# PaulTFLi/Machine-Learning-Replications

Hardware: AMD Instinct MI355X
Metric: train_rows_per_sec (higher is better)
Workload: dtype fp32

## Files before the change

### machine-learning-replications_amd/models/imputer.py

```python
from __future__ import annotations

import os

import numpy as np
import torch

from .base import Estimator, as_tensor

SLOTS = 8
MFMA_FILTER = os.environ.get("HFENS_KNN_MFMA", "auto")
MFMA_MIN_PAIRS = 1 << 24
EXACT = __import__("os").environ.get("HFENS_KNN_EXACT", "1") != "0"
KNN_DEBUG = __import__("os").environ.get("HFENS_KNN_DEBUG", "0") == "1"
DEVICE_PLAN = __import__("os").environ.get("HFENS_KNN_DEVICE_PLAN", "1") != "0"
LAST_REFINE: list = []
REFINE_CAP_MIN = 1 << 18
REFINE_CAP_PER_ROW = 16


def _refine_debug(work, cap, nr, Mx):
    o = 4 * cap + 8 * nr * SLOTS + 2 * nr
    LAST_REFINE.append((nr, int(work[o]), int(work[o + 8]), int(work[o + 9]), int(work[o + 4]), float(Mx[0])))


def _masks_u64(miss: torch.Tensor) -> torch.Tensor:
    F = miss.shape[1]
    w = (2 ** torch.arange(F, dtype=torch.int64, device=miss.device))
    bits = (miss.to(torch.int64) * w).sum(1)
    return bits


class KNNImputer(Estimator):
    _param_names = ("missing_values", "n_neighbors", "weights", "metric", "copy")

    def __init__(self, missing_values=np.nan, n_neighbors=5, weights="uniform", metric="nan_euclidean",
                 copy=True):
        self.missing_values = missing_values
        self.n_neighbors = n_neighbors
        self.weights = weights
        self.metric = metric
        self.copy = copy

    def fit(self, X):
        X = as_tensor(X)
        self._fit_X = X
        self._mask_fit = torch.isnan(X)
        self._valid = ~self._mask_fit.all(0)
        fx = torch.where(self._mask_fit, torch.zeros_like(X), X)
        cnt = (~self._mask_fit).sum(0).clamp(min=1)
        self._col_mean = fx.sum(0) / cnt
        self._keep_host = None
        return self

    def _keep(self):
        if self._keep_host is None:
            self._keep_host = np.nonzero(self._valid.cpu().numpy())[0].astype(np.int64)
        return self._keep_host

    def fit_transform(self, X):
        return self.fit(X).transform(X)

    def transform(self, X):
        return self.transform_many([X])[0]

    def transform_many(self, Xs, streams=None, defer=False):
        Xs = [as_tensor(X, device=self._fit_X.device).clone() for X in Xs]
        if Xs and Xs[0].is_cuda and self.n_neighbors == 1:
            if DEVICE_PLAN and EXACT and Xs[0].shape[1] <= 64:
                return self._impute_planned_many(Xs, streams, defer)
            return self._impute_device_many(Xs, streams, defer)
        if defer:
            done = self.transform_many(Xs)
            return done, (lambda: done)
        for X in Xs:
            miss = torch.isnan(X)
            rows = torch.nonzero(miss.any(1)).squeeze(1)
            if rows.numel() > 0:
                self._impute_host(X, miss, rows)
        return [X[:, self._valid] for X in Xs]

    def _fit_prep(self):
        pr = getattr(self, "_prep", None)
        if pr is None or pr[0] is not self._fit_X:
            D = torch.where(self._mask_fit, torch.zeros_like(self._fit_X), self._fit_X)
            center = self._col_mean
            D32 = (D - center).where(~self._mask_fit, torch.zeros_like(D)).to(torch.float32).contiguous()
            dm = _masks_u64(self._mask_fit).contiguous()
            D64 = D.to(torch.float64).contiguous()
            dmax = D32.abs().amax(0) if D32.numel() else torch.zeros(D32.shape[1], device=D.device)
            pr = self._prep = (self._fit_X, D32, dm, D64, dmax)
        return pr[1], pr[2]

    def _fit_prep64(self):
        self._fit_prep()
        return self._prep[3], self._prep[4]

    def _impute_planned_many(self, Xs, streams, defer=False):
        from .smo import _to_dev
        from ..utils.timing import hmark
        dev = Xs[0].device
        F = Xs[0].shape[1]
        keep_h = self._keep()
        keep = None if keep_h.shape[0] == F else _to_dev(keep_h, dev)
        D32, dm = self._fit_prep()
        D64, dmax = self._fit_prep64()
        main = torch.cuda.current_stream(dev)
        ready = torch.cuda.Event()
        ready.record(main)
        out, jobs = [], []
        for i, X in enumerate(Xs):
            st = streams[i] if streams is not None and streams[i] is not None else None
            if st is None:
                self._impute_planned(X, D32, dm, D64, dmax)
                out.append(X if keep is None else X.index_select(1, keep))
                hmark("imp_main_enqueued")
            else:
                def job(i=i, X=X, st=st):
                    st.wait_event(ready)
                    for t in (X, D32, dm, D64, dmax, self._fit_X, self._col_mean) + ((keep,) if keep is not None else ()):
                        t.record_stream(st)
                    with torch.cuda.device(dev), torch.cuda.stream(st):
                        self._impute_planned(X, D32, dm, D64, dmax)
                        out[i] = X if keep is None else X.index_select(1, keep)
                out.append(None)
                jobs.append(job)
        if not defer:
            for job in jobs:
                job()
            return out
        state = {"done": False}

        def run():
            if not state["done"]:
                for job in jobs:
                    job()
                state["done"] = True
            return out
        return out, run

    def _impute_planned(self, X, D32, dm, D64, dmax):
        from .. import ops
        E = ops.ext()
        n, F = X.shape
        if n == 0:
            return
        dev = X.device
        s = ops.stream_ptr(dev)
        G = -(-F // SLOTS)
        Xc = X if X.is_contiguous() else X.contiguous()
        i64, i32 = torch.int64, torch.int32
        rows = torch.empty(n, dtype=i64, device=dev)
        rbits = torch.empty(n, dtype=i64, device=dev)
        slot = torch.empty(G, n, SLOTS, dtype=i32, device=dev)
        R32 = torch.empty(n, F, dtype=torch.float32, device=dev)
        R64 = torch.empty(n, F, dtype=torch.float64, device=dev)
        small = torch.empty(F + 1 + 4 + (n + 255) // 256, dtype=i32, device=dev)
        colmax, Mx, cnt, bcnt = small[:F], small[F:F + 1], small[F + 1:F + 5], small[F + 5:]
        E.knn_plan_dev(Xc.data_ptr(), n, F, self._col_mean.data_ptr(), dmax.data_ptr(), rows.data_ptr(),
                       rbits.data_ptr(), slot.data_ptr(), G, R32.data_ptr(), R64.data_ptr(), colmax.data_ptr(),
                       Mx.data_ptr(), cnt.data_ptr(), bcnt.data_ptr(), s)
        best = torch.empty(G, n, SLOTS, dtype=i64, device=dev)
        alt = torch.empty(n, SLOTS, dtype=i32, device=dev)
        cap = max(REFINE_CAP_MIN, REFINE_CAP_PER_ROW * n, 1)
        work = torch.empty(4 * cap + n * SLOTS * 8 + 2 * n + 12, dtype=i32, device=dev)
        nd = D32.shape[0]
        mf = None
        use_mf = MFMA_FILTER == "1" or (MFMA_FILTER == "auto" and n * nd >= MFMA_MIN_PAIRS)
        if use_mf and F <= 48 and nd > 0:
            wd = np.zeros(1, dtype=np.int64)
            E.knn_mfma_item_words(F, wd.ctypes.data)
            mf = (torch.empty(nd * int(wd[0]), dtype=torch.int32, device=dev), torch.empty(nd, dtype=torch.float32, device=dev))
            E.knn_mfma_prep(D32.data_ptr(), dm.data_ptr(), nd, F, mf[0].data_ptr(), mf[1].data_ptr(), s)
        for g in range(G):
            if mf is not None:
                E.knn_donors_mfma(R32.data_ptr(), rbits.data_ptr(), n, D32.data_ptr(), dm.data_ptr(), nd, F,
                                  slot[g].data_ptr(), best[g].data_ptr(), alt.data_ptr(), cnt.data_ptr(), g * SLOTS,
                                  mf[0].data_ptr(), mf[1].data_ptr(), s)
            else:
                E.knn_donors(R32.data_ptr(), rbits.data_ptr(), n, D32.data_ptr(), dm.data_ptr(), nd, F,
                             slot[g].data_ptr(), best[g].data_ptr(), alt.data_ptr(), cnt.data_ptr(), g * SLOTS, s)
            E.knn_refine(R32.data_ptr(), rbits.data_ptr(), n, D32.data_ptr(), dm.data_ptr(), nd, F,
                         slot[g].data_ptr(), best[g].data_ptr(), alt.data_ptr(), R64.data_ptr(), D64.data_ptr(),
                         Mx.data_ptr(), work.data_ptr(), cap, cnt.data_ptr(), g * SLOTS,
                         mf[0].data_ptr() if mf is not None else 0, mf[1].data_ptr() if mf is not None else 0, s)
            if KNN_DEBUG:
                _refine_debug(work, cap, n, Mx)
        fx = self._fit_X if self._fit_X.is_contiguous() else self._fit_X.contiguous()
        E.knn_apply(Xc.data_ptr(), n, F, rows.data_ptr(), slot.data_ptr(), best.data_ptr(), fx.data_ptr(),
                    self._col_mean.data_ptr(), cnt.data_ptr(), s)
        if Xc is not X:
            X.copy_(Xc)

    def _impute_device_many(self, Xs, streams, defer=False):
        F = Xs[0].shape[1]
        if F > 64:
            raise ValueError("KNNImputer device path supports at most 64 features")
        from ..utils.timing import hmark
        host = torch.cat([_masks_u64(torch.isnan(X)) for X in Xs] + [self._valid.to(torch.int64)]).cpu().numpy()
        hmark("imp_masks_read")
        bits_all = host[:-F].view(np.uint64)
        from .smo import _to_dev
        dev = Xs[0].device
        keep = _to_dev(np.nonzero(host[-F:])[0].astype(np.int64), dev)
        D32, dm = self._fit_prep()
        main = torch.cuda.current_stream(dev)
        ready = torch.cuda.Event()
        ready.record(main)
        off, out, jobs = 0, [], []
        for i, X in enumerate(Xs):
            bits = bits_all[off:off + X.shape[0]]
            off += X.shape[0]
            st = streams[i] if streams is not None and streams[i] is not None else None
            if st is None:
                self._impute_device(X, bits, D32, dm)
                out.append(X.index_select(1, keep))
                hmark("imp_main_enqueued")
            else:
                def job(i=i, X=X, bits=bits, st=st):
                    st.wait_event(ready)
                    for t in (X, keep, D32, dm, self._fit_X, self._col_mean):
                        t.record_stream(st)
                    with torch.cuda.device(dev), torch.cuda.stream(st):
                        self._impute_device(X, bits, D32, dm)
                        out[i] = X.index_select(1, keep)
                out.append(None)
                jobs.append(job)
        if not defer:
            for job in jobs:
                job()
            return out
        state = {"done": False}

        def run():
            if not state["done"]:
                for job in jobs:
                    job()
                state["done"] = True
            return out
        return out, run

    def _impute_device(self, X, bits, D32, dm):
        from .. import ops
        E = ops.ext()
        n, F = X.shape
        dev = X.device
        dims = np.zeros(4, dtype=np.int64)
        bits = np.ascontiguousarray(bits, dtype=np.uint64)
        E.knn_plan_host(bits.ctypes.data, n, F, SLOTS, 0, 0, dims.ctypes.data)
        nr, nc, nslot = (int(v) for v in dims[:3])
        if nr == 0:
            return
        cap = 2 * nr + nr * nslot + 3 * nc
        hb = torch.empty(cap, dtype=torch.int64, pin_memory=True)
        E.knn_plan_host(bits.ctypes.data, n, F, SLOTS, hb.data_ptr(), cap, dims.ctypes.data)
        if int(dims[3]) != 0 or int(dims[0]) != nr:
            raise RuntimeError(f"knn_plan_host: work-list buffer of {cap} words rejected (dims {dims.tolist()})")
        center = self._col_mean
        from ..utils.timing import hmark
        hmark("imp_plan")
        sizes = [nr, nr, nr * nslot, nc, nc, nc]
        buf = hb[:sum(sizes)].to(dev, non_blocking=True)
        o = np.concatenate([[0], np.cumsum(sizes)])
        rows, rm, slot_dev, flat, r_idx, c_idx = (buf[o[i]:o[i + 1]] for i in range(6))
        hmark("imp_h2d")
        Rm = ((rm[:, None] >> torch.arange(F, device=dev)) & 1) != 0
        slot_dev = slot_dev.view(nr, nslot).to(torch.int32)
        Xr = X.index_select(0, rows)
        R32 = torch.where(Rm, torch.zeros_like(Xr), Xr - center).to(torch.float32).contiguous()
        rm = rm.contiguous()
        best = torch.empty(nr, nslot, dtype=torch.int64, device=dev)
        alt = torch.empty(nr, SLOTS, dtype=torch.int32, device=dev)
        if EXACT:
            D64, dmax = self._fit_prep64()
            R64 = torch.where(Rm, torch.zeros_like(Xr), Xr).to(torch.float64).contiguous()
            Mx = torch.linalg.vector_norm(torch.maximum(dmax, R32.abs().amax(0)).to(torch.float64)).reshape(1)
            Mx = Mx.to(torch.float32).contiguous()
            cap = max(REFINE_CAP_MIN, REFINE_CAP_PER_ROW * nr, 1)
            work = torch.empty(4 * cap + nr * SLOTS * 8 + 2 * nr + 12, dtype=torch.int32, device=dev)
        for s0 in range(0, nslot, SLOTS):
            slot = slot_dev[:, s0:s0 + SLOTS].contiguous()
            blk = best[:, s0:s0 + SLOTS] if nslot == SLOTS else torch.empty(slot.shape, dtype=torch.int64, device=dev)
            E.knn_donors(R32.data_ptr(), rm.data_ptr(), nr, D32.data_ptr(), dm.data_ptr(),
                         D32.shape[0], F, slot.data_ptr(), blk.data_ptr(), alt.data_ptr(), 0, 0, ops.stream_ptr(dev))
            if EXACT:
                E.knn_refine(R32.data_ptr(), rm.data_ptr(), nr, D32.data_ptr(), dm.data_ptr(), D32.shape[0], F,
                             slot.data_ptr(), blk.data_ptr(), alt.data_ptr(), R64.data_ptr(), D64.data_ptr(),
                             Mx.data_ptr(), work.data_ptr(), cap, 0, 0, 0, 0, ops.stream_ptr(dev))
                if KNN_DEBUG:
                    _refine_debug(work, cap, nr, Mx)
            if nslot != SLOTS:
                best[:, s0:s0 + SLOTS] = blk
        hmark("imp_knn_launched")
        b = best.view(-1).index_select(0, flat)
        donor = torch.where(b == -1, torch.full_like(b, -1), b & 0xFFFFFFFF)
        vals = torch.where(donor >= 0, self._fit_X[donor.clamp(min=0), c_idx], self._col_mean[c_idx])
        X.index_put_((r_idx, c_idx), vals)

    def _impute_host(self, X, miss, rows):
        fit = self._fit_X
        mf = self._mask_fit
        F = X.shape[1]
        D = torch.where(mf, torch.zeros_like(fit), fit)
        pres_f = (~mf).to(torch.float64)
        step = max(1, (1 << 24) // max(1, fit.shape[0] * F))
        for s in range(0, rows.numel(), step):
            rr = rows[s:s + step]
            R = X[rr]
            mr = torch.isnan(R)
            Rz = torch.where(mr, torch.zeros_like(R), R)
            pres_r = (~mr).to(torch.float64)
            both = pres_r[:, None, :] * pres_f[None, :, :]
            diff = Rz[:, None, :] - D[None, :, :]
            sq = both * (diff * diff)
            d2 = sq[..., 0].clone()
            for f in range(1, F):
                d2 = d2 + sq[..., f]
            common = both.sum(-1)
            dist = torch.where(common > 0, d2 * F / common.clamp(min=1),
                               torch.full_like(d2, float("inf")))
            for j, r in enumerate(rr.tolist()):
                for c in torch.nonzero(mr[j]).squeeze(1).tolist():
                    cand = ~mf[:, c]
                    dd = torch.where(cand, dist[j], torch.full_like(dist[j], float("inf")))
                    k = min(self.n_neighbors, int(cand.sum()))
                    if k == 0 or not torch.isfinite(dd).any():
                        X[r, c] = self._col_mean[c]
                        continue
                    if k == 1:
                        X[r, c] = fit[int(torch.argmin(dd)), c]
                        continue
                    vals, idx = torch.topk(-dd, k)
                    ok = torch.isfinite(vals)
                    X[r, c] = fit[idx[ok], c].mean()
```

### machine-learning-replications_amd/ops/csrc/decls.inc

```
#if defined(HFENS_DECLS)
#define HFENS_OP(name, sig) void name sig;
#elif defined(HFENS_DEFS)
#define HFENS_OP(name, sig) m.def(#name, &hfens::name);
#endif
HFENS_OP(gbdt_apply_prep, (int B, int n, int F, int NN, uintptr_t bins, uintptr_t y, uintptr_t w,
                           uintptr_t raw, uintptr_t g, uintptr_t h, uintptr_t node, uintptr_t prev_feat,
                           uintptr_t prev_blo, uintptr_t prev_value, uintptr_t prev_r2,
                           uintptr_t dev_acc, uintptr_t cur_r2, double lr, double qscale,
                           double dscale, uintptr_t wt, double subsample, uintptr_t seeds,
                           long long row_off, int stage, uintptr_t stream))
HFENS_OP(gbdt_hist, (int B, int n, int F, uintptr_t bins, uintptr_t nbins, int max_nb, uintptr_t g,
                     uintptr_t h, uintptr_t w, uintptr_t node, int node0, int NL, uintptr_t hist,
                     double qscale, uintptr_t stream))
HFENS_OP(gbdt_split, (int B, int F, int NN, uintptr_t hist, uintptr_t nbins, uintptr_t lo_val,
                      uintptr_t hi_val, int node0, int NL, int last_level, double min_leaf_q,
                      double min_split_q, double qscale, uintptr_t feat, uintptr_t blo, uintptr_t thr,
                      uintptr_t value, uintptr_t stats, uintptr_t r2, uintptr_t stream))
HFENS_OP(gbdt_route, (int B, int n, int NN, uintptr_t bins, uintptr_t g, uintptr_t w, uintptr_t node,
                      uintptr_t feat, uintptr_t blo, uintptr_t r2, int node0, int NL, double qscale,
                      uintptr_t stream))
HFENS_OP(gbdt_stumps_fused, (int B, int n, int F, int T, uintptr_t bins, uintptr_t nbins, int hist_len,
                             uintptr_t lo_val, uintptr_t hi_val, uintptr_t y, uintptr_t w, uintptr_t raw,
                             uintptr_t g, uintptr_t h, uintptr_t wt, uintptr_t seeds, long long row_off,
                             double subsample, uintptr_t feat, uintptr_t blo, uintptr_t thr, uintptr_t value,
                             uintptr_t stats, uintptr_t r2, uintptr_t dev, uintptr_t bagw, double lr,
                             double qscale, double dscale, double min_leaf_q, double min_split_q,
                             uintptr_t stream))
HFENS_OP(l1_qp_cd, (int B, int F1, uintptr_t H, uintptr_t g, uintptr_t w, uintptr_t penal, double lam,
                    int max_sweeps, double tol, uintptr_t d_out, uintptr_t stream))
HFENS_OP(logreg_fused, (int B, int n, int F1, uintptr_t X, uintptr_t s, uintptr_t ypm, uintptr_t penal, double C,
                        int l1, int max_outer, uintptr_t Z, uintptr_t Xd, uintptr_t W, uintptr_t iters,
                        uintptr_t stream))
HFENS_OP(logreg_coop, (int B, int members, int n, int F1, uintptr_t X, uintptr_t s, uintptr_t ypm, uintptr_t penal,
                       double C, int l1, int max_outer, uintptr_t Z, uintptr_t Xd, uintptr_t W, uintptr_t iters,
                       uintptr_t xchg, uintptr_t err, uintptr_t stream))
HFENS_OP(lasso_cd_path, (int P, int F, int A, uintptr_t G, uintptr_t q, uintptr_t yy, uintptr_t nrows,
                         uintptr_t alphas, int max_iter, double tol, uintptr_t coefs, uintptr_t gaps,
                         uintptr_t iters, uintptr_t stream))
HFENS_OP(gram_rbf_batch, (uintptr_t Z, int F, uintptr_t probs, int P, int max_l, uintptr_t K,
                          uintptr_t stream))
HFENS_OP(smo_batch, (uintptr_t probs, int P, int max_l, uintptr_t K, uintptr_t alpha, double eps,
                     long long max_iter, uintptr_t rho, uintptr_t iters, uintptr_t gap, uintptr_t prof,
                     uintptr_t stream))
HFENS_OP(coop_resident_blocks, (uintptr_t out))
HFENS_OP(smo_coop_batch, (uintptr_t probs, int P, int W, int max_S, uintptr_t K, uintptr_t maps,
                          uintptr_t alpha, uintptr_t xchg, double eps, long long max_iter, uintptr_t rho,
                          uintptr_t iters, uintptr_t gap, uintptr_t err, uintptr_t prof, uintptr_t stream))
HFENS_OP(smo_coop_otf_batch, (uintptr_t probs, int P, int W, int F, int max_S, uintptr_t zcat, uintptr_t alpha,
                              uintptr_t xchg, double eps, long long max_iter, uintptr_t rho, uintptr_t iters,
                              uintptr_t gap, uintptr_t err, uintptr_t stream))
HFENS_OP(platt_batch,(uintptr_t probs, int P, uintptr_t part, int S, uintptr_t rowk, uintptr_t rho,
                       uintptr_t consts, uintptr_t srcmap, uintptr_t dec, uintptr_t AB, uintptr_t coop_bar,
                       uintptr_t coop_part, uintptr_t stream))
HFENS_OP(knn_mfma_item_words, (int F, uintptr_t out))
HFENS_OP(knn_mfma_prep, (uintptr_t D, uintptr_t dmask, int nd, int F, uintptr_t items, uintptr_t ny, uintptr_t stream))
HFENS_OP(knn_donors_mfma, (uintptr_t R, uintptr_t rmask, int nr, uintptr_t D, uintptr_t dmask, int nd, int F,
                           uintptr_t slot_col, uintptr_t best, uintptr_t alt, uintptr_t cnt, int s0, uintptr_t items,
                           uintptr_t ny, uintptr_t stream))
HFENS_OP(knn_donors, (uintptr_t R, uintptr_t rmask, int nr, uintptr_t D, uintptr_t dmask, int nd, int F,
                      uintptr_t slot_col, uintptr_t best, uintptr_t alt, uintptr_t cnt, int s0, uintptr_t stream))
HFENS_OP(knn_plan_host, (uintptr_t bits_, long long n, int F, int slots, uintptr_t out_, long long cap,
                         uintptr_t dims_))
HFENS_OP(knn_refine, (uintptr_t R, uintptr_t rmask, int nr, uintptr_t D, uintptr_t dmask, int nd, int F,
                      uintptr_t slot_col, uintptr_t best, uintptr_t alt, uintptr_t R64, uintptr_t D64, uintptr_t Mx,
                      uintptr_t work, long long cap, uintptr_t cnt, int s0, uintptr_t items, uintptr_t ny,
                      uintptr_t stream))
HFENS_OP(weighted_moments, (uintptr_t X, int n, int F, uintptr_t W, uintptr_t V, int P, uintptr_t Gpart,
                            uintptr_t apart, uintptr_t vpart, uintptr_t stream))
HFENS_OP(svc_oof, (uintptr_t dec, uintptr_t model, uintptr_t rho, uintptr_t AB, uintptr_t rows, uintptr_t meta,
                   int ld, int col, int n, uintptr_t stream))
HFENS_OP(svm_dec_batch, (uintptr_t zcat, uintptr_t coef, uintptr_t hcat, int F, uintptr_t probs, int P,
                         int max_h, int S, uintptr_t part, uintptr_t counts, uintptr_t stream))
HFENS_OP(svm_sv_compact, (uintptr_t zcat, uintptr_t coef, int F, uintptr_t probs, int P, uintptr_t zc, uintptr_t cc,
                          uintptr_t counts, uintptr_t stream))
HFENS_OP(libsvm_perm, (int l, long long seed, uintptr_t out_ptr))
HFENS_OP(svc_expand_host, (uintptr_t y_ptr, long long n, long long seed, uintptr_t out_ptr, uintptr_t meta_ptr))
HFENS_OP(sklearn_stump_ranks, (int T, int F, uintptr_t seeds_ptr, uintptr_t constant_ptr, uintptr_t ranks_ptr))
HFENS_OP(wsyrk_f64, (uintptr_t Phi, uintptr_t d, long long n, int r, uintptr_t part, long long part_len, uintptr_t S,
                     uintptr_t stream))
HFENS_OP(wsyrk_f32, (uintptr_t Phi, uintptr_t d, long long n, int r, uintptr_t part, long long part_len, uintptr_t S,
                     uintptr_t stream))
HFENS_OP(wsyrk_f64x, (uintptr_t Phi, uintptr_t d, long long n, int r, uintptr_t part, long long part_len, uintptr_t S,
                      uintptr_t stream))
HFENS_OP(phi_gemv, (uintptr_t Phi, uintptr_t W, long long n, int r, int k, uintptr_t Y, uintptr_t stream))
HFENS_OP(fill_dev, (uintptr_t out, long long n, uintptr_t src, uintptr_t stream))
HFENS_OP(ipm_max_step, (uintptr_t v0, uintptr_t d0, uintptr_t v1, uintptr_t d1, uintptr_t v2, uintptr_t d2,
                        uintptr_t v3, uintptr_t d3, double s0, double s1, double s2, double s3, long long n,
                        uintptr_t out, uintptr_t stream))
HFENS_OP(scale_rows_f32, (uintptr_t P, uintptr_t d, long long n, int r, uintptr_t out, uintptr_t stream))
HFENS_OP(ipm_resid, (uintptr_t c, uintptr_t a, uintptr_t y, uintptr_t P, int sp, uintptr_t b, uintptr_t nu, uintptr_t mu,
                     long long n, uintptr_t s, uintptr_t rd, uintptr_t stream))
HFENS_OP(ipm_pred, (uintptr_t a, uintptr_t s, uintptr_t nu, uintptr_t mu, uintptr_t rd, uintptr_t y, long long n,
                    uintptr_t Dinv, uintptr_t Dinv2, uintptr_t rnu, uintptr_t rmu, uintptr_t H2, uintptr_t stream))
HFENS_OP(ipm_corr, (uintptr_t a, uintptr_t s, uintptr_t nu, uintptr_t mu, uintptr_t da, uintptr_t dnu, uintptr_t dmu,
                    uintptr_t rd, uintptr_t tau, long long n, uintptr_t rnu, uintptr_t rmu, uintptr_t h, uintptr_t stream))
HFENS_OP(ipm_minv_pre, (uintptr_t Dinv, uintptr_t y, uintptr_t U, int k, long long n, uintptr_t du, uintptr_t V,
                        uintptr_t stream))
HFENS_OP(ipm_minv_post, (uintptr_t Dinv, uintptr_t y, uintptr_t du, uintptr_t P, int k, long long n, uintptr_t out,
                         uintptr_t stream))
HFENS_OP(ipm_update, (uintptr_t a, uintptr_t nu, uintptr_t mu, uintptr_t da, uintptr_t dnu, uintptr_t dmu, uintptr_t t,
                      long long n, uintptr_t a2, uintptr_t nu2, uintptr_t mu2, uintptr_t stream))
HFENS_OP(ipm_dirs, (uintptr_t Mh, int smh, uintptr_t My, int smy, uintptr_t db, uintptr_t rnu, uintptr_t rmu,
                    uintptr_t nu, uintptr_t mu, uintptr_t a, uintptr_t s, long long n, uintptr_t da, uintptr_t dnu,
                    uintptr_t dmu, uintptr_t stream))
HFENS_OP(ipm_gondzio_rhs, (uintptr_t a, uintptr_t s, uintptr_t nu, uintptr_t mu, uintptr_t da, uintptr_t dnu,
                           uintptr_t dmu, uintptr_t alpha, uintptr_t tau, long long n, uintptr_t ta, uintptr_t ts,
                           uintptr_t rhs, uintptr_t stream))
HFENS_OP(ipm_gondzio_apply, (uintptr_t Mh, int smh, uintptr_t My, int smy, uintptr_t dbc, uintptr_t da,
                             uintptr_t dnu, uintptr_t dmu, uintptr_t ta, uintptr_t ts, uintptr_t nu, uintptr_t mu,
                             uintptr_t a, uintptr_t s, long long n, uintptr_t nda, uintptr_t ndnu, uintptr_t ndmu,
                             uintptr_t stream))
HFENS_OP(ipm_select3, (uintptr_t ok, uintptr_t x0, uintptr_t x1, uintptr_t x2, long long n, uintptr_t y0,
                       uintptr_t y1, uintptr_t y2, uintptr_t stream))
HFENS_OP(phi_gemv_f32, (uintptr_t Phi, uintptr_t W, long long n, int r, int k, uintptr_t Y, uintptr_t stream))
HFENS_OP(phit_f32, (uintptr_t Phi, uintptr_t V, long long n, int r, int k, uintptr_t part, long long part_len,
                    uintptr_t out, uintptr_t stream))
HFENS_OP(scaler_batch, (uintptr_t X, long long n, int F, uintptr_t rows, uintptr_t offs, int K, long long max_rows,
                        uintptr_t part, uintptr_t mean, uintptr_t var, uintptr_t Z, uintptr_t stream))
HFENS_OP(chol_spd, (uintptr_t S, int r, uintptr_t L, uintptr_t sc, uintptr_t info, uintptr_t stream))
HFENS_OP(chol_spd_mw, (uintptr_t S, int r, uintptr_t L, uintptr_t sc, uintptr_t info, uintptr_t work, uintptr_t PT,
                       uintptr_t stream))
HFENS_OP(chol_solve, (uintptr_t L, uintptr_t sc, int r, int k, uintptr_t B, uintptr_t stream))
HFENS_OP(gbdt_stage_tick, (uintptr_t t_dev, uintptr_t stream))
HFENS_OP(gbdt_stump_stage, (int t, int B, int n, int F, int T, uintptr_t bins, long long ldb, uintptr_t nbins, int hist_len,
                            uintptr_t lo_val, uintptr_t hi_val, uintptr_t y, uintptr_t w, uintptr_t raw,
                            uintptr_t wt, uintptr_t seeds, long long row_off, double subsample, uintptr_t comm,
                            uintptr_t feat, uintptr_t blo, uintptr_t thr, uintptr_t value, uintptr_t stats,
                            uintptr_t r2, uintptr_t dev, uintptr_t bagw, uintptr_t frank, uintptr_t partials,
                            long long partials_len, double lr, double qscale, double dscale,
                            double min_leaf_q, double min_split_q, uintptr_t prof, uintptr_t t_dev,
                            int tick_in_reduce, int persist, uintptr_t bar, uintptr_t err, uintptr_t stream))
HFENS_OP(stack_infer, (uintptr_t X, int x_f64, long long n, int F, int mp, int T, int K, double ngl2e,
                       double svc_b, double probA, double probB, double gb_init, double gb_lr,
                       double lr_b, double mw0, double mw1, double mw2, double mb, uintptr_t mean,
                       uintptr_t inv_scale, uintptr_t svt, uintptr_t sn, uintptr_t coef,
                       uintptr_t nodes, uintptr_t values, uintptr_t lr_w, uintptr_t st_off,
                       uintptr_t st_pairs, double st_base, uintptr_t out, int grid, uintptr_t stream))
HFENS_OP(stack_coalition, (uintptr_t X, long long n, uintptr_t BG, long long B, int F, int mp, int T, int K,
                           double ngl2e, double svc_b, double probA, double probB, double gb_init,
                           double gb_lr, double lr_b, double mw0, double mw1, double mw2, double mb,
                           uintptr_t mean, uintptr_t inv_scale, uintptr_t svt, uintptr_t sn, uintptr_t coef,
                           uintptr_t nodes, uintptr_t values, uintptr_t lr_w, uintptr_t st_off,
                           uintptr_t st_pairs, double st_base, uintptr_t v, int grid, uintptr_t stream))
HFENS_OP(shapley_reduce, (uintptr_t v, long long n, int F, uintptr_t w, uintptr_t phi, uintptr_t stream))
HFENS_OP(ws_init, (uintptr_t probs, int P, int max_l, uintptr_t zcat, int F, uintptr_t zn, uintptr_t alpha,
                   uintptr_t G, uintptr_t states, uintptr_t keys, long long n, uintptr_t hist, uintptr_t gkey,
                   uintptr_t stream))
HFENS_OP(cascade_where, (uintptr_t tab, int Q, long long max_len, uintptr_t where, uintptr_t stream))
HFENS_OP(ws_seed, (uintptr_t probs, int P, int max_l, uintptr_t zcat, int F, uintptr_t zn, uintptr_t aseed,
                   uintptr_t alpha, uintptr_t G, uintptr_t keys, long long n, uintptr_t gkey, uintptr_t stream))
HFENS_OP(ws_steps, (uintptr_t probs, int P, int max_l, uintptr_t zcat, int F, uintptr_t zn, uintptr_t alpha,
                    uintptr_t G, uintptr_t states, uintptr_t wsz, uintptr_t wsn, uintptr_t wdc, uintptr_t wsprev,
                    uintptr_t wsidx, uintptr_t keys, long long n, uintptr_t gkey, double eps, int max_outer, int max_inner,
                    double inner_frac, int n_iter, uintptr_t prof, int inner_threads, int q, uintptr_t stream))
HFENS_OP(ws_steps_kc, (uintptr_t probs, int P, int max_l, uintptr_t zcat, int F, uintptr_t zn, uintptr_t alpha,
                       uintptr_t G, uintptr_t states, uintptr_t wsz, uintptr_t wsn, uintptr_t wdc, uintptr_t wsprev,
                       uintptr_t keys, long long n, uintptr_t gkey, uintptr_t cand, double eps, int max_outer,
                       int max_inner, double inner_frac, int n_iter, uintptr_t prof, uintptr_t stream))
HFENS_OP(ws_kc_cand_len, (long long max_l, uintptr_t out))
HFENS_OP(ws_finalize, (uintptr_t probs, int P, uintptr_t states, uintptr_t alpha, uintptr_t G, uintptr_t rho,
                       uintptr_t iters, uintptr_t inner, uintptr_t gap, uintptr_t stream))
HFENS_OP(binned_stump_raw, (uintptr_t bins, long long n, int F, uintptr_t tables, int B, uintptr_t init,
                            uintptr_t out, uintptr_t stream))
HFENS_OP(forest_fp8, (uintptr_t bins, long long ldb, long long n, int F, int T, int d, uintptr_t nodes, uintptr_t bfrag,
                      int Q, int S, uintptr_t inv_scale, uintptr_t init, uintptr_t out, uintptr_t stream))
HFENS_OP(quantize_bins, (uintptr_t X, int f64, long long n, int F, uintptr_t edges, int K, uintptr_t nbins,
                         uintptr_t out, long long ldb, uintptr_t stream))
HFENS_OP(stack_predict_host, (int n, int F, uintptr_t X_, uintptr_t mean_, uintptr_t scale_, int nsv, uintptr_t sv_,
                              uintptr_t coef_, double gamma, double svc_icpt, double probA, double probB, int T,
                              int K, uintptr_t feat_, uintptr_t thr_, uintptr_t left_, uintptr_t right_,
                              uintptr_t value_, double gbc_init, double lr, uintptr_t lrc_, double lr_icpt,
                              uintptr_t meta_, double meta_icpt, uintptr_t out_))
HFENS_OP(wsyrk_part_len, (long long n, int r, uintptr_t out))
HFENS_OP(phit_part_len, (long long n, int r, int k, uintptr_t out))
HFENS_OP(gbdt_stage_plan, (long long n, int B, int hist_len, int ncu, uintptr_t out))
HFENS_OP(xgmi_alloc, (long long bytes, int uncached, uintptr_t out))
HFENS_OP(xgmi_free, (uintptr_t p))
HFENS_OP(xgmi_ipc_handle, (uintptr_t p, uintptr_t out))
HFENS_OP(xgmi_ipc_open, (uintptr_t handle, uintptr_t out))
HFENS_OP(xgmi_ipc_close, (uintptr_t p))
HFENS_OP(xgmi_allreduce, (uintptr_t local, long long count, int dtype, int op, uintptr_t peers, int W, int me,
                          int k, long long cap, long long epoch_base, int t_host, uintptr_t t_dev, uintptr_t err,
                          double timeout_s, uintptr_t stream))
HFENS_OP(xgmi_allreduce_i64, (uintptr_t local, long long count, uintptr_t peers, int W, int me, int k, long long cap,
                              long long epoch_base, int t_host, uintptr_t t_dev, uintptr_t err, double timeout_s,
                              uintptr_t stream))
HFENS_OP(gbdt_ranks_dev, (int T, int B, int F, int n, uintptr_t bins, long long ldb, uintptr_t w, uintptr_t seeds,
                          uintptr_t ranks, uintptr_t stream))
HFENS_OP(oof_trees, (uintptr_t X, int F, uintptr_t rows, uintptr_t model, long long m, int T, int B, int NN,
                     uintptr_t feat, uintptr_t thr, uintptr_t value, uintptr_t init, double lr, uintptr_t meta, int ld,
                     int col, uintptr_t stream))
HFENS_OP(oof_linear, (uintptr_t X, int F, uintptr_t rows, uintptr_t model, long long m, uintptr_t W, int F1,
                      int has_icpt, double icpt_scale, uintptr_t meta, int ld, int col, uintptr_t stream))
HFENS_OP(svm_gamma, (uintptr_t Z, uintptr_t offs, int K, int F, uintptr_t gamma, uintptr_t ngl2e, uintptr_t stream))
HFENS_OP(svm_patch_f32, (uintptr_t base, int stride, int off, int count, uintptr_t fit_of, uintptr_t src,
                         uintptr_t stream))
HFENS_OP(knn_plan_dev, (uintptr_t X, long long n, int F, uintptr_t centre, uintptr_t dmax, uintptr_t rows,
                        uintptr_t rbits, uintptr_t slot, int G, uintptr_t R32, uintptr_t R64, uintptr_t colmax,
                        uintptr_t Mx, uintptr_t cnt, uintptr_t bcnt, uintptr_t stream))
HFENS_OP(knn_apply, (uintptr_t X, long long n, int F, uintptr_t rows, uintptr_t slot, uintptr_t best, uintptr_t fitX,
                     uintptr_t colmean, uintptr_t cnt, uintptr_t stream))
HFENS_OP(host_store, (uintptr_t src, uintptr_t dst_host, long long n, int elem_bytes, uintptr_t stream))
HFENS_OP(rbf_f64, (uintptr_t Z, long long l, uintptr_t L, int m, int F, double gamma, uintptr_t out, uintptr_t stream))
#undef HFENS_OP
```

### machine-learning-replications_amd/ops/csrc/knn.hip

```cpp
#include "common.h"
#include <cstdlib>
#include <type_traits>

namespace hfens {

constexpr int kKnnTile = 256;
constexpr int kKnnSlots = 8;

__device__ __forceinline__ void knn_merge_slots(unsigned long long* best, unsigned* alt, int r,
                                                const float (&bd)[kKnnSlots], const float (&b2)[kKnnSlots],
                                                const int (&bi)[kKnnSlots]) {
#pragma unroll
  for (int k = 0; k < kKnnSlots; ++k) {
    if (bi[k] < 0) continue;
    const size_t e = (size_t)r * kKnnSlots + k;
    const unsigned long long key =
        ((unsigned long long)__float_as_uint(bd[k]) << 32) | (unsigned long long)(unsigned)bi[k];
    const unsigned long long old = atomicMin(&best[e], key);
    const unsigned long long loser = old < key ? key : old;
    if (loser != ~0ull) atomicMin(&alt[e], (unsigned)(loser >> 32));
    if (b2[k] < INFINITY) atomicMin(&alt[e], __float_as_uint(b2[k]));
  }
}

template <int FMAX>
__global__ __launch_bounds__(256) void knn_donor_kernel(
    const float* __restrict__ R, const unsigned long long* __restrict__ rmask, int nr,
    const float* __restrict__ D, const unsigned long long* __restrict__ dmask, int nd, int F,
    int per_split, const int* __restrict__ slot_col ,
    unsigned long long* __restrict__ best ,
    unsigned* __restrict__ alt ,
    const int* __restrict__ cnt , int s0) {
  if (cnt != nullptr) {
    if (s0 >= cnt[1]) return;
    nr = cnt[0];
  }
  constexpr int LD = (FMAX + 3) / 4 * 4;
  extern __shared__ __attribute__((aligned(16))) float sm[];
  float* ds = sm;
  unsigned long long* dm = (unsigned long long*)(ds + kKnnTile * LD);
  const int r = blockIdx.x * 256 + threadIdx.x;
  const bool active = r < nr;
  const int d_begin = blockIdx.y * per_split;
  const int d_end = min(nd, d_begin + per_split);
  float xr[LD];
#pragma unroll
  for (int f = 0; f < LD; ++f) xr[f] = (active && f < F) ? R[(size_t)r * F + f] : 0.f;
  const unsigned long long mr = active ? rmask[r] : 0ull;
  int col[kKnnSlots];
  float bd[kKnnSlots], b2[kKnnSlots];
  int bi[kKnnSlots];
  bool any = false;
#pragma unroll
  for (int k = 0; k < kKnnSlots; ++k) {
    col[k] = active ? slot_col[(size_t)r * kKnnSlots + k] : -1;
    bd[k] = INFINITY;
    b2[k] = INFINITY;
    bi[k] = -1;
    any |= col[k] >= 0;
  }
  unsigned long long need = 0ull;
#pragma unroll
  for (int k = 0; k < kKnnSlots; ++k)
    if (col[k] >= 0) need |= 1ull << col[k];
  float bmax = INFINITY;
  for (int d0 = d_begin; d0 < d_end; d0 += kKnnTile) {
    __syncthreads();
    const int nt = min(kKnnTile, d_end - d0);
    for (int e = threadIdx.x; e < nt * LD; e += 256) {
      const int rr = e / LD, c = e % LD;
      ds[e] = c < F ? D[(size_t)(d0 + rr) * F + c] : 0.f;
    }
    if (threadIdx.x < nt) dm[threadIdx.x] = dmask[d0 + threadIdx.x];
    __syncthreads();
    if (!any) continue;
    for (int t = 0; t < nt; ++t) {
      const unsigned long long md = dm[t];
      if ((need & ~md) == 0ull) continue;
      const float4* xd4 = reinterpret_cast<const float4*>(ds + t * LD);
      const unsigned long long both = ~(mr | md);
      const unsigned blo = (unsigned)both, bhi = (unsigned)(both >> 32);
      float s0 = 0.f, s1 = 0.f;
#pragma unroll
      for (int q = 0; q < LD / 4; ++q) {
        if (4 * q < F) {
          const float4 v = xd4[q];
          const unsigned bq = ((4 * q < 32 ? blo >> (4 * q) : bhi >> (4 * q - 32))) & 0xFu;
          const float a = (bq & 1u) ? xr[4 * q] - v.x : 0.f;
          const float b = (bq & 2u) ? xr[4 * q + 1] - v.y : 0.f;
          const float c = (bq & 4u) ? xr[4 * q + 2] - v.z : 0.f;
          const float d = (bq & 8u) ? xr[4 * q + 3] - v.w : 0.f;
          s0 = fmaf(a, a, s0);
          s1 = fmaf(b, b, s1);
          s0 = fmaf(c, c, s0);
          s1 = fmaf(d, d, s1);
        }
      }
      const float s = s0 + s1;
      const int present = F - __builtin_popcountll(mr | md);
      if (present <= 0) continue;
      const float dist = fmaxf(s, 0.f) * ((float)F / (float)present);
      if (!(dist < bmax)) continue;
      const int di = d0 + t;
      float m = 0.f;
#pragma unroll
      for (int k = 0; k < kKnnSlots; ++k) {
        if (col[k] >= 0 && !((md >> col[k]) & 1ull) && dist < b2[k]) {
          const bool nb = dist < bd[k];
          b2[k] = nb ? bd[k] : dist;
          bi[k] = nb ? di : bi[k];
          bd[k] = nb ? dist : bd[k];
        }
        if (col[k] >= 0) m = fmaxf(m, b2[k]);
      }
      bmax = m;
    }
  }
  if (active) knn_merge_slots(best, alt, r, bd, b2, bi);
}

constexpr int kKnnFastTile = 224;
template <int FMAX>
constexpr bool knn_fast_xs() { return (FMAX + 3) / 4 * 4 <= 40; }
template <int FMAX>
constexpr int knn_fast_tile() { return knn_fast_xs<FMAX>() ? kKnnFastTile : kKnnTile; }

template <int FMAX>
constexpr size_t knn_fast_lds() {
  constexpr int LD = (FMAX + 3) / 4 * 4;
  return (size_t)knn_fast_tile<FMAX>() * LD * sizeof(float) + knn_fast_tile<FMAX>() * sizeof(unsigned long long) +
         (knn_fast_xs<FMAX>() ? (size_t)LD * 256 * sizeof(float) : 0);
}
template <int FMAX>
constexpr size_t knn_fast_lds_sm() {
  return knn_fast_xs<FMAX>() ? (size_t)((FMAX + 3) / 4 * 4) * 256 * sizeof(float) : 0;
}

template <int FMAX, bool SM>
__global__ __launch_bounds__(256) void knn_donor_fast_kernel(
    const float* __restrict__ R, const unsigned long long* __restrict__ rmask, int nr,
    const float* __restrict__ D, const unsigned long long* __restrict__ dmask, int nd, int F,
    int per_split, const int* __restrict__ slot_col, unsigned long long* __restrict__ best,
    unsigned* __restrict__ alt, const int* __restrict__ cnt, int s0) {
  if (cnt != nullptr) {
    if (s0 >= cnt[1]) return;
    nr = cnt[0];
  }
  constexpr int LD = (FMAX + 3) / 4 * 4;
  constexpr bool XS = knn_fast_xs<FMAX>();
  constexpr int TILE = knn_fast_tile<FMAX>();
  typedef float f32x2v __attribute__((ext_vector_type(2)));
  extern __shared__ __attribute__((aligned(16))) float sm[];
  float* ds = sm;
  unsigned long long* dm = (unsigned long long*)(ds + (SM ? 0 : TILE * LD));
  float* xs = SM ? sm : reinterpret_cast<float*>(dm + TILE);
  const int r = blockIdx.x * 256 + threadIdx.x;
  const bool active = r < nr;
  const int d_begin = blockIdx.y * per_split;
  const int d_end = min(nd, d_begin + per_split);
  const unsigned long long mr = active ? rmask[r] : 0ull;
  f32x2v xr2[LD / 2], nm2[LD / 2];
#pragma unroll
  for (int h = 0; h < LD / 2; ++h) {
    xr2[h] = f32x2v{(active && 2 * h < F) ? R[(size_t)r * F + 2 * h] : 0.f,
                    (active && 2 * h + 1 < F) ? R[(size_t)r * F + 2 * h + 1] : 0.f};
    const float m0 = (2 * h < F && !((mr >> (2 * h)) & 1ull)) ? -1.f : -0.f;
    const float m1 = (2 * h + 1 < F && !((mr >> (2 * h + 1)) & 1ull)) ? -1.f : -0.f;
    nm2[h] = f32x2v{m0, m1};
    if constexpr (XS) {
      xs[(2 * h) * 256 + threadIdx.x] = xr2[h][0];
      xs[(2 * h + 1) * 256 + threadIdx.x] = xr2[h][1];
    }
  }
  int col[kKnnSlots];
  float bd[kKnnSlots], b2[kKnnSlots];
  int bi[kKnnSlots];
  bool any = false;
#pragma unroll
  for (int k = 0; k < kKnnSlots; ++k) {
    col[k] = active ? slot_col[(size_t)r * kKnnSlots + k] : -1;
    bd[k] = INFINITY;
    b2[k] = INFINITY;
    bi[k] = -1;
    any |= col[k] >= 0;
  }
  unsigned long long need = 0ull;
#pragma unroll
  for (int k = 0; k < kKnnSlots; ++k)
    if (col[k] >= 0) need |= 1ull << col[k];
  float bmax = INFINITY;
  __shared__ float s_scale[65];
  if (threadIdx.x <= 64) s_scale[threadIdx.x] = threadIdx.x > 0 ? (float)F / (float)threadIdx.x : 0.f;
  for (int d0 = d_begin; d0 < d_end; d0 += TILE) {
    const int nt = min(TILE, d_end - d0);
    if constexpr (SM) {
      __syncthreads();
    } else {
    __syncthreads();
    if (XS && F == LD) {
      const float4* src = reinterpret_cast<const float4*>(D + (size_t)d0 * F);
      float4* dst = reinterpret_cast<float4*>(ds);
      const int n4 = nt * LD / 4;
      constexpr int U = XS ? (TILE * LD / 4 + 255) / 256 : 0, UC = 4;
#pragma unroll
      for (int u0 = 0; u0 < U; u0 += UC) {
        float4 v[UC];
#pragma unroll
        for (int u = 0; u < UC; ++u) {
          const int e = threadIdx.x + 256 * (u0 + u);
          v[u] = (u0 + u < U && e < n4) ? src[e] : make_float4(0.f, 0.f, 0.f, 0.f);
        }
#pragma unroll
        for (int u = 0; u < UC; ++u) {
          const int e = threadIdx.x + 256 * (u0 + u);
          if (u0 + u < U && e < n4) dst[e] = v[u];
        }
      }
    } else {
      for (int e = threadIdx.x; e < nt * LD; e += 256) {
        const int rr = e / LD, c = e % LD;
        ds[e] = c < F ? D[(size_t)(d0 + rr) * F + c] : 0.f;
      }
    }
    if (threadIdx.x < nt) dm[threadIdx.x] = dmask[d0 + threadIdx.x];
    __syncthreads();
    }
    if (!any) continue;
    auto donor = [&](int t, float sf) {
      const unsigned long long md = SM ? dmask[d0 + t] : dm[t];
      if ((need & ~md) == 0ull) return;
      const int present = F - __builtin_popcountll(mr | md);
      if (present <= 0) return;
      const float scale = s_scale[present];
      const bool exact = md == 0ull;
      if (!exact) {
        float corr = 0.f;
        unsigned long long mm = md & ~mr & ((F >= 64) ? ~0ull : ((1ull << F) - 1ull));
        while (mm) {
          const int f = __builtin_ctzll(mm);
          mm &= mm - 1ull;
          float xv = 0.f;
          if constexpr (XS) {
            xv = xs[f * 256 + threadIdx.x];
          } else {
#pragma unroll
            for (int g = 0; g < LD; ++g) xv = g == f ? xr2[g >> 1][g & 1] : xv;
          }
          corr = fmaf(xv, xv, corr);
        }
        const float lb = (sf - corr) - 1.52587890625e-05f * (sf + corr);
        if (!(fmaxf(lb, 0.f) * scale * 0.99999905f < bmax)) return;
      } else if (!(fmaxf(sf, 0.f) * scale < bmax)) {
        return;
      }
      float s = sf;
      if (!exact) {
        const float4* xd4 = SM ? reinterpret_cast<const float4*>(D + (size_t)(d0 + t) * LD)
                               : reinterpret_cast<const float4*>(ds + t * LD);
        const unsigned long long both = ~(mr | md);
        const unsigned blo = (unsigned)both, bhi = (unsigned)(both >> 32);
        float s0 = 0.f, s1 = 0.f;
#pragma unroll
        for (int q = 0; q < LD / 4; ++q) {
          const float4 v = xd4[q];
          const unsigned bq = ((4 * q < 32 ? blo >> (4 * q) : bhi >> (4 * q - 32))) & 0xFu;
          const float a = (bq & 1u) ? xr2[2 * q][0] - v.x : 0.f;
          const float b = (bq & 2u) ? xr2[2 * q][1] - v.y : 0.f;
          const float c = (bq & 4u) ? xr2[2 * q + 1][0] - v.z : 0.f;
          const float d = (bq & 8u) ? xr2[2 * q + 1][1] - v.w : 0.f;
          s0 = fmaf(a, a, s0);
          s1 = fmaf(b, b, s1);
          s0 = fmaf(c, c, s0);
          s1 = fmaf(d, d, s1);
        }
        s = s0 + s1;
      }
      const float dist = fmaxf(s, 0.f) * scale;
      if (!(dist < bmax)) return;
      const int di = d0 + t;
      float m = 0.f;
#pragma unroll
      for (int k = 0; k < kKnnSlots; ++k) {
        if (col[k] >= 0 && !((md >> col[k]) & 1ull) && dist < b2[k]) {
          const bool nb = dist < bd[k];
          b2[k] = nb ? bd[k] : dist;
          bi[k] = nb ? di : bi[k];
          bd[k] = nb ? dist : bd[k];
        }
        if (col[k] >= 0) m = fmaxf(m, b2[k]);
      }
      bmax = m;
    };
    for (int t = 0; t < nt; t += 2) {
      const int t1 = t + 1 < nt ? t + 1 : t;
      const float4* xa = SM ? reinterpret_cast<const float4*>(D + (size_t)(d0 + t) * LD)
                            : reinterpret_cast<const float4*>(ds + t * LD);
      const float4* xb = SM ? reinterpret_cast<const float4*>(D + (size_t)(d0 + t1) * LD)
                            : reinterpret_cast<const float4*>(ds + t1 * LD);
      f32x2v accA = f32x2v{0.f, 0.f}, accB = f32x2v{0.f, 0.f};
#pragma unroll
      for (int q = 0; q < LD / 4; ++q) {
        const float4 va = xa[q], vb = xb[q];
        const f32x2v a0 = __builtin_elementwise_fma(nm2[2 * q], f32x2v{va.x, va.y}, xr2[2 * q]);
        const f32x2v a1 = __builtin_elementwise_fma(nm2[2 * q + 1], f32x2v{va.z, va.w}, xr2[2 * q + 1]);
        const f32x2v b0 = __builtin_elementwise_fma(nm2[2 * q], f32x2v{vb.x, vb.y}, xr2[2 * q]);
        const f32x2v b1 = __builtin_elementwise_fma(nm2[2 * q + 1], f32x2v{vb.z, vb.w}, xr2[2 * q + 1]);
        accA = __builtin_elementwise_fma(a0, a0, accA);
        accB = __builtin_elementwise_fma(b0, b0, accB);
        accA = __builtin_elementwise_fma(a1, a1, accA);
        accB = __builtin_elementwise_fma(b1, b1, accB);
      }
      donor(t, accA.x + accA.y);
      if (t1 != t) donor(t1, accB.x + accB.y);
    }
  }
  if (active) knn_merge_slots(best, alt, r, bd, b2, bi);
}

void knn_donors(uintptr_t R, uintptr_t rmask, int nr, uintptr_t D, uintptr_t dmask, int nd, int F,
                uintptr_t slot_col, uintptr_t best, uintptr_t alt, uintptr_t cnt, int s0, uintptr_t stream) {
  HFENS_REQUIRE(F >= 1 && F <= 64, "knn_donors: 1 <= F <= 64 (64-bit missing masks)");
  if (nr == 0 || nd == 0) return;
  hipStream_t st = as_stream(stream);
  HFENS_CHECK(hipMemsetAsync((void*)best, 0xFF, (size_t)nr * kKnnSlots * sizeof(unsigned long long), st));
  HFENS_CHECK(hipMemsetAsync((void*)alt, 0xFF, (size_t)nr * kKnnSlots * sizeof(unsigned), st));
  const int rb = (nr + 255) / 256;
  int splits = 2048 / rb;
  const int by_range = (nd + 16383) / 16384;
  if (splits < by_range) splits = by_range;
  const int max_splits = (nd + kKnnTile - 1) / kKnnTile;
  if (splits > max_splits) splits = max_splits;
  if (splits < 1) splits = 1;
  const char* kenv = std::getenv("HFENS_KNN_KERNEL");
  const bool direct = kenv && kenv[0] == 'd';
  const bool lds_tiles = kenv && kenv[0] == 'l';
  auto go = [&](auto fm) {
    constexpr int FM = decltype(fm)::value;
    constexpr int LD = (FM + 3) / 4 * 4;
    const int tile = direct ? kKnnTile : knn_fast_tile<FM>();
    int per = (nd + splits - 1) / splits;
    per = (per + tile - 1) / tile * tile;
    const int nsp = (nd + per - 1) / per;
    const size_t lds = direct ? (size_t)kKnnTile * LD * sizeof(float) + kKnnTile * sizeof(unsigned long long)
                              : knn_fast_lds<FM>();
    if (direct)
      hipLaunchKernelGGL(knn_donor_kernel<FM>, dim3(rb, nsp), dim3(256), lds, st, (const float*)R,
                         (const unsigned long long*)rmask, nr, (const float*)D,
                         (const unsigned long long*)dmask, nd, F, per, (const int*)slot_col,
                         (unsigned long long*)best, (unsigned*)alt, (const int*)cnt, s0);
    else if (F == LD && !lds_tiles && (D & 15) == 0)
      hipLaunchKernelGGL((knn_donor_fast_kernel<FM, true>), dim3(rb, nsp), dim3(256), knn_fast_lds_sm<FM>(), st,
                         (const float*)R, (const unsigned long long*)rmask, nr, (const float*)D,
                         (const unsigned long long*)dmask, nd, F, per, (const int*)slot_col,
                         (unsigned long long*)best, (unsigned*)alt, (const int*)cnt, s0);
    else
      hipLaunchKernelGGL((knn_donor_fast_kernel<FM, false>), dim3(rb, nsp), dim3(256), lds, st, (const float*)R,
                         (const unsigned long long*)rmask, nr, (const float*)D,
                         (const unsigned long long*)dmask, nd, F, per, (const int*)slot_col,
                         (unsigned long long*)best, (unsigned*)alt, (const int*)cnt, s0);
    launch_check();
  };
  if (F <= 16) go(std::integral_constant<int, 16>{});
  else if (F <= 32) go(std::integral_constant<int, 32>{});
  else if (F <= 40) go(std::integral_constant<int, 40>{});
  else if (F <= 48) go(std::integral_constant<int, 48>{});
  else go(std::integral_constant<int, 64>{});
}


template <int FM>
struct KnnMf {
  static constexpr int NB = (7 * FM + 15) / 16;
  static constexpr int LP = NB * 16;
  static constexpr int LPS = LP + 8;
  static constexpr int TILE = 32;
  static constexpr int WAVES = FM >= 48 ? 4 : 8;
  static constexpr int A4 = TILE * LP / 8;
  static constexpr int Y4 = TILE * FM / 4;
};
typedef __bf16 knn_bf16x8 __attribute__((ext_vector_type(8)));
typedef unsigned int knn_u32x4 __attribute__((ext_vector_type(4)));

__device__ __forceinline__ unsigned knn_bf_hi(float v) { return __float_as_uint(v) >> 16; }
__device__ __forceinline__ unsigned knn_bf_lo(float v) {
  const float r = v - __uint_as_float(__float_as_uint(v) & 0xFFFF0000u);
  return __float_as_uint(r) >> 16;
}

template <int FM>
__global__ __launch_bounds__(256) void knn_mfma_prep_kernel(const float* __restrict__ D,
                                                            const unsigned long long* __restrict__ dmask,
                                                            int nd, int F, unsigned short* __restrict__ items,
                                                            float* __restrict__ rowsFM, float* __restrict__ ny) {
  using K = KnnMf<FM>;
  const int d = blockIdx.x * blockDim.x + threadIdx.x;
  if (d >= nd) return;
  const unsigned long long md = dmask[d];
  unsigned short* it = items + (size_t)d * K::LP;
  float nsum = 0.f;
  for (int f = 0; f < FM; ++f) {
    const float y = (f < F && !((md >> f) & 1ull)) ? D[(size_t)d * F + f] : 0.f;
    rowsFM[(size_t)d * FM + f] = y;
    nsum = fmaf(y, y, nsum);
  }
  for (int q = 0; q < K::LP; ++q) {
    const int kind = q / FM, f = q - kind * FM;
    const bool miss = f >= F || ((md >> f) & 1ull);
    const float y = miss ? 0.f : D[(size_t)d * F + f];
    unsigned w = 0u;
    if (kind <= 1) w = knn_bf_hi(y);
    else if (kind == 2) w = knn_bf_lo(y);
    else if (kind <= 4) w = (f < F && miss) ? 0x3F80u : 0u;
    else if (kind == 5) w = knn_bf_hi(y * y);
    else if (kind == 6) w = knn_bf_lo(y * y);
    it[q] = (unsigned short)w;
  }
  ny[d] = nsum;
}

template <int FM, int MODE = 0>
__global__ __launch_bounds__(512) void knn_donor_mfma_kernel(
    const float* __restrict__ R, const unsigned long long* __restrict__ rmask, int nr,
    const float* __restrict__ rowsFM, const unsigned long long* __restrict__ dmask, int nd, int F,
    int per_split, const int* __restrict__ slot_col, unsigned long long* __restrict__ best,
    unsigned* __restrict__ alt, const int* __restrict__ cnt, int s0,
    const unsigned short* __restrict__ items, const float* __restrict__ ny_all,
    const int* __restrict__ rlist = nullptr, const float* __restrict__ thr = nullptr,
    int* __restrict__ pairs = nullptr, long long cap = 0, int* __restrict__ pcount = nullptr) {
  using K = KnnMf<FM>;
  if constexpr (MODE == 1) {
    nr = cnt[0];
    if ((int)blockIdx.x * (32 * K::WAVES) >= nr) return;
  } else if (cnt != nullptr) {
    if (s0 >= cnt[1]) return;
    nr = cnt[0];
  }
  constexpr int LD = FM;
  constexpr int NT = 64 * K::WAVES;
  __shared__ __attribute__((aligned(16))) unsigned short tA[K::TILE * K::LPS];
  __shared__ __attribute__((aligned(16))) float tY[K::TILE * LD];
  __shared__ unsigned long long tM[K::TILE];
  __shared__ knn_u32x4 tR[K::TILE];
  __shared__ __attribute__((aligned(16))) float tNy[K::TILE];
  __shared__ float s_scale[65];
  const int tid = threadIdx.x, wave = tid >> 6, lane = tid & 63, r32 = lane & 31, hh = lane >> 5;
  const int li = blockIdx.x * (32 * K::WAVES) + wave * 32 + r32;
  const bool active = li < nr;
  const int r = MODE == 1 ? (active ? rlist[li] : 0) : li;
  const int d_begin = blockIdx.y * per_split;
  const int d_end = min(nd, d_begin + per_split);
  const unsigned long long mr = active ? rmask[r] : 0ull;
  __shared__ __attribute__((aligned(16))) float xs[32 * K::WAVES][LD + 4];
  __shared__ unsigned long long smr[32 * K::WAVES];
  constexpr int kQc = 16;
  __shared__ unsigned short clist[K::WAVES][64 * kQc];
  __shared__ int q_idx[K::WAVES][64][kQc];
  __shared__ float q_dist[K::WAVES][64][kQc];
  float* xrow = xs[wave * 32 + r32];
  if (hh == 0) smr[wave * 32 + r32] = mr;
  float nx = 0.f;
  for (int f = hh; f < LD; f += 2) {
    const float v = (active && f < F && !((mr >> f) & 1ull)) ? R[(size_t)r * F + f] : 0.f;
    xrow[f] = v;
  }
  __syncthreads();
#pragma unroll 8
  for (int f = 0; f < LD; ++f) nx = fmaf(xrow[f], xrow[f], nx);
  knn_bf16x8 bq[K::NB];
#pragma unroll
  for (int m = 0; m < K::NB; ++m) {
    unsigned w[4];
#pragma unroll
    for (int e2 = 0; e2 < 4; ++e2) {
      unsigned v2[2];
#pragma unroll
      for (int dd = 0; dd < 2; ++dd) {
        const int q = 16 * m + 8 * hh + 2 * e2 + dd;
        const int kind = q / FM, f = q - kind * FM;
        const float xv = kind < 7 ? xrow[f] : 0.f;
        const float v = kind <= 2 ? -2.f * xv : -(xv * xv);
        const bool rm = f < F && ((mr >> f) & 1ull);
        unsigned ww = 0u;
        if (kind == 0 || kind == 2 || kind == 3) ww = knn_bf_hi(v);
        else if (kind == 1 || kind == 4) ww = knn_bf_lo(v);
        else if (kind <= 6) ww = rm ? 0xBF80u : 0u;
        v2[dd] = ww;
      }
      w[e2] = v2[0] | (v2[1] << 16);
    }
    bq[m] = __builtin_bit_cast(knn_bf16x8, (knn_u32x4){w[0], w[1], w[2], w[3]});
  }
  int col[kKnnSlots];
  float bd[kKnnSlots], b2[kKnnSlots];
  int bi[kKnnSlots];
  bool any = false;
  float tmax = -1.f;
#pragma unroll
  for (int k = 0; k < kKnnSlots; ++k) {
    const size_t e = (size_t)r * kKnnSlots + k;
    bd[k] = INFINITY;
    b2[k] = INFINITY;
    bi[k] = -1;
    if constexpr (MODE == 1) {
      const float t = active ? thr[e] : -1.f;
      col[k] = t >= 0.f ? slot_col[e] : -1;
      b2[k] = t;
      if (col[k] >= 0) tmax = fmaxf(tmax, t);
    } else {
      col[k] = active ? slot_col[e] : -1;
    }
    any |= col[k] >= 0;
  }
  unsigned long long need = 0ull;
#pragma unroll
  for (int k = 0; k < kKnnSlots; ++k)
    if (col[k] >= 0) need |= 1ull << col[k];
  float bmax = MODE == 1 ? (tmax >= 0.f ? tmax * 1.00000095f : -1.f) : INFINITY;
  if (tid <= 64) s_scale[tid] = tid > 0 ? (float)F / (float)tid : 0.f;
  const float fF = (float)F * 0.99999905f;
  const bool wave_any = __ballot(any) != 0ull;
  constexpr int PA = (K::A4 + NT - 1) / NT, PY = (K::Y4 + NT - 1) / NT;
  knn_u32x4 pa[PA];
  float4 py[PY];
  unsigned long long pm = ~0ull;
  float pn = 0.f;
  auto fetch = [&](int d0) {
    const int nt = min(K::TILE, d_end - d0);
    const knn_u32x4* srcA = reinterpret_cast<const knn_u32x4*>(items + (size_t)d0 * K::LP);
    const float4* srcY = reinterpret_cast<const float4*>(rowsFM + (size_t)d0 * LD);
#pragma unroll
    for (int u = 0; u < PA; ++u) {
      const int e = tid + u * NT;
      pa[u] = (e < nt * K::LP / 8) ? srcA[e] : (knn_u32x4){0u, 0u, 0u, 0u};
    }
#pragma unroll
    for (int u = 0; u < PY; ++u) {
      const int e = tid + u * NT;
      py[u] = (e < nt * LD / 4) ? srcY[e] : make_float4(0.f, 0.f, 0.f, 0.f);
    }
    if (tid < K::TILE) {
      pm = tid < nt ? dmask[d0 + tid] : ~0ull;
      pn = tid < nt ? ny_all[d0 + tid] : 0.f;
    }
  };
  int qlen = 0;
  auto flush = [&]() {
    const int mine = qlen;
    int incl = mine;
#pragma unroll
    for (int o = 1; o < 64; o <<= 1) {
      const int v = __shfl_up(incl, o, 64);
      if (lane >= o) incl += v;
    }
    const int total = __shfl(incl, 63, 64);
    if (total == 0) return;
    for (int e = 0, pos = incl - mine; e < mine; ++e, ++pos) clist[wave][pos] = (unsigned short)((lane << 5) | e);
    __builtin_amdgcn_fence(__ATOMIC_RELEASE, "wavefront");
    __builtin_amdgcn_wave_barrier();
    __builtin_amdgcn_fence(__ATOMIC_ACQUIRE, "wavefront");
    for (int c = lane; c < total; c += 64) {
      const int code = clist[wave][c];
      const int owner = code >> 5, e = code & 31;
      const int di = q_idx[wave][owner][e];
      const unsigned long long md = dmask[di];
      const unsigned long long mro = smr[wave * 32 + (owner & 31)];
      const int present = F - __builtin_popcountll(mro | md);
      const float4* xd4 = reinterpret_cast<const float4*>(rowsFM + (size_t)di * LD);
      const float4* xr4 = reinterpret_cast<const float4*>(xs[wave * 32 + (owner & 31)]);
      const unsigned long long both = ~(mro | md);
      const unsigned blo = (unsigned)both, bhi = (unsigned)(both >> 32);
      float sa = 0.f, sb = 0.f;
#pragma unroll
      for (int q = 0; q < LD / 4; ++q) {
        const float4 v = xd4[q];
        const float4 u = xr4[q];
        const unsigned bqm = ((4 * q < 32 ? blo >> (4 * q) : bhi >> (4 * q - 32))) & 0xFu;
        const float a = (bqm & 1u) ? u.x - v.x : 0.f;
        const float b = (bqm & 2u) ? u.y - v.y : 0.f;
        const float cc = (bqm & 4u) ? u.z - v.z : 0.f;
        const float d = (bqm & 8u) ? u.w - v.w : 0.f;
        sa = fmaf(a, a, sa);
        sb = fmaf(b, b, sb);
        sa = fmaf(cc, cc, sa);
        sb = fmaf(d, d, sb);
      }
      q_dist[wave][owner][e] = fmaxf(sa + sb, 0.f) * s_scale[present];
    }
    __builtin_amdgcn_fence(__ATOMIC_RELEASE, "wavefront");
    __builtin_amdgcn_wave_barrier();
    __builtin_amdgcn_fence(__ATOMIC_ACQUIRE, "wavefront");
    for (int e = 0; e < mine; ++e) {
      const float dist = q_dist[wave][lane][e];
      if constexpr (MODE == 1) {
        const int di = q_idx[wave][lane][e];
        const unsigned long long md = dmask[di];
#pragma unroll
        for (int k = 0; k < kKnnSlots; ++k) {
          if (col[k] >= 0 && !((md >> col[k]) & 1ull) && dist <= b2[k]) {
            const int p = atomicAdd(&pcount[0], 1);
            if (p < cap) {
              pairs[2 * (size_t)p] = (int)((size_t)r * kKnnSlots + k);
              pairs[2 * (size_t)p + 1] = di;
            } else {
              pcount[1] = 1;
            }
          }
        }
        continue;
      }
      if (!(dist < bmax)) continue;
      const int di = q_idx[wave][lane][e];
      const unsigned long long md = dmask[di];
      float mx = 0.f;
#pragma unroll
      for (int k = 0; k < kKnnSlots; ++k) {
        if (col[k] >= 0 && !((md >> col[k]) & 1ull) && dist < b2[k]) {
          const bool nb = dist < bd[k];
          b2[k] = nb ? bd[k] : dist;
          bi[k] = nb ? di : bi[k];
          bd[k] = nb ? dist : bd[k];
        }
        if (col[k] >= 0) mx = fmaxf(mx, b2[k]);
      }
      bmax = mx;
    }
    qlen = 0;
    __builtin_amdgcn_wave_barrier();
  };
  if (d_begin < d_end) fetch(d_begin);
  for (int d0 = d_begin; d0 < d_end; d0 += K::TILE) {
    const int nt = min(K::TILE, d_end - d0);
    __syncthreads();
#pragma unroll
    for (int u = 0; u < PA; ++u) {
      const int e = tid + u * NT;
      if (e < K::A4) reinterpret_cast<knn_u32x4*>(tA)[(e / (K::LP / 8)) * (K::LPS / 8) + e % (K::LP / 8)] = pa[u];
    }
#pragma unroll
    for (int u = 0; u < PY; ++u) {
      const int e = tid + u * NT;
      if (e < K::Y4) reinterpret_cast<float4*>(tY)[e] = py[u];
    }
    if (tid < K::TILE) {
      tM[tid] = pm;
      tR[tid] = (knn_u32x4){(unsigned)pm, (unsigned)(pm >> 32), __float_as_uint(pn), 0u};
      tNy[tid] = pn;
    }
    __syncthreads();
    if (d0 + K::TILE < d_end) fetch(d0 + K::TILE);
    if (!wave_any) continue;
    f32x16 acc = {0.f};
#pragma unroll
    for (int m = 0; m < K::NB; ++m) {
      const knn_u32x4 raw = *reinterpret_cast<const knn_u32x4*>(&tA[r32 * K::LPS + 16 * m + 8 * hh]);
      acc = __builtin_amdgcn_mfma_f32_32x32x16_bf16(__builtin_bit_cast(knn_bf16x8, raw), bq[m], acc, 0, 0, 0);
    }
    unsigned cand = 0u;
    if (any) {
      const float bq1 = bmax * 1.0000038f;
      const float nxk = nx * 0.99951171875f;
      unsigned pre = 0u;
#pragma unroll
      for (int g = 0; g < 4; ++g) {
        const float4 ny4 = *reinterpret_cast<const float4*>(&tNy[8 * g + 4 * hh]);
        pre |= (unsigned)(fmaf(ny4.x, 0.99951171875f, nxk) + acc[4 * g] < bq1) << (4 * g);
        pre |= (unsigned)(fmaf(ny4.y, 0.99951171875f, nxk) + acc[4 * g + 1] < bq1) << (4 * g + 1);
        pre |= (unsigned)(fmaf(ny4.z, 0.99951171875f, nxk) + acc[4 * g + 2] < bq1) << (4 * g + 2);
        pre |= (unsigned)(fmaf(ny4.w, 0.99951171875f, nxk) + acc[4 * g + 3] < bq1) << (4 * g + 3);
      }
      while (pre) {
        const int j = __builtin_ctz(pre);
        pre &= pre - 1u;
        const int row = (j & 3) + 8 * (j >> 2) + 4 * hh;
        const knn_u32x4 rw = *reinterpret_cast<const knn_u32x4*>(&tR[row]);
        const unsigned long long md = (unsigned long long)rw.x | ((unsigned long long)rw.y << 32);
        const float ynorm = __uint_as_float(rw.z);
        const int present = F - __builtin_popcountll(mr | md);
        float aj = 0.f;
#pragma unroll
        for (int jj = 0; jj < 16; ++jj) aj = jj == j ? acc[jj] : aj;
        const float lhs = fmaxf((nx + ynorm) + aj - 4.8828125e-04f * (nx + ynorm), 0.f) * fF;
        const bool ok = ((need & ~md) != 0ull) & (present > 0) & (lhs < bmax * (float)present);
        cand |= (unsigned)ok << j;
      }
    }
    if (__ballot(cand != 0u) == 0ull) continue;
    if (__ballot(qlen + __builtin_popcount(cand) > kQc) != 0ull) flush();
    while (cand) {
      const int j = __builtin_ctz(cand);
      cand &= cand - 1u;
      q_idx[wave][lane][qlen++] = d0 + (j & 3) + 8 * (j >> 2) + 4 * hh;
    }
  }
  flush();
  if constexpr (MODE == 0)
    if (active) knn_merge_slots(best, alt, r, bd, b2, bi);
}

static int knn_mf_fm(int F) { return F <= 16 ? 16 : F <= 24 ? 24 : F <= 32 ? 32 : F <= 40 ? 40 : 48; }
void knn_mfma_item_words(int F, uintptr_t out) {
  const int FM = knn_mf_fm(F);
  *reinterpret_cast<long long*>(out) = (long long)(((7 * FM + 15) / 16) * 16 / 2 + FM);
}

void knn_mfma_prep(uintptr_t D, uintptr_t dmask, int nd, int F, uintptr_t items, uintptr_t ny, uintptr_t stream) {
  HFENS_REQUIRE(F >= 1 && F <= 48, "knn_mfma_prep: 1 <= F <= 48");
  if (nd == 0) return;
  auto go = [&](auto fm) {
    constexpr int FM = decltype(fm)::value;
    using K = KnnMf<FM>;
    unsigned short* it = (unsigned short*)items;
    float* rows = reinterpret_cast<float*>(it + (size_t)nd * K::LP);
    hipLaunchKernelGGL(knn_mfma_prep_kernel<FM>, dim3((nd + 255) / 256), dim3(256), 0, as_stream(stream),
                       (const float*)D, (const unsigned long long*)dmask, nd, F, it, rows, (float*)ny);
  };
  const int FM = knn_mf_fm(F);
  if (FM == 16) go(std::integral_constant<int, 16>{});
  else if (FM == 24) go(std::integral_constant<int, 24>{});
  else if (FM == 32) go(std::integral_constant<int, 32>{});
  else if (FM == 40) go(std::integral_constant<int, 40>{});
  else go(std::integral_constant<int, 48>{});
  launch_check();
}

void knn_donors_mfma(uintptr_t R, uintptr_t rmask, int nr, uintptr_t D, uintptr_t dmask, int nd, int F,
                     uintptr_t slot_col, uintptr_t best, uintptr_t alt, uintptr_t cnt, int s0, uintptr_t items,
                     uintptr_t ny, uintptr_t stream) {
  HFENS_REQUIRE(F >= 1 && F <= 48, "knn_donors_mfma: 1 <= F <= 48");
  (void)D;
  if (nr == 0 || nd == 0) return;
  hipStream_t st = as_stream(stream);
  HFENS_CHECK(hipMemsetAsync((void*)best, 0xFF, (size_t)nr * kKnnSlots * sizeof(unsigned long long), st));
  HFENS_CHECK(hipMemsetAsync((void*)alt, 0xFF, (size_t)nr * kKnnSlots * sizeof(unsigned), st));
  const int rpb = knn_mf_fm(F) >= 48 ? 128 : 256;
  const int rb = (nr + rpb - 1) / rpb;
  static const int kWgs = getenv("HFENS_KNN_MFMA_WGS") ? atoi(getenv("HFENS_KNN_MFMA_WGS")) : 256;
  static const int kMinPer = getenv("HFENS_KNN_MFMA_MINPER") ? atoi(getenv("HFENS_KNN_MFMA_MINPER")) : 256;
  static const int kRange = getenv("HFENS_KNN_MFMA_RANGE") ? atoi(getenv("HFENS_KNN_MFMA_RANGE")) : (1 << 30);
  int splits = kWgs / rb;
  const int by_range = (nd + kRange - 1) / kRange;
  if (splits < by_range) splits = by_range;
  const int max_splits = (nd + kMinPer - 1) / kMinPer;
  if (splits > max_splits) splits = max_splits;
  if (splits < 1) splits = 1;
  int per = (nd + splits - 1) / splits;
  per = (per + 31) / 32 * 32;
  const int nsp = (nd + per - 1) / per;
  auto go = [&](auto fm) {
    constexpr int FM = decltype(fm)::value;
    using K = KnnMf<FM>;
    const unsigned short* it = (const unsigned short*)items;
    const float* rows = reinterpret_cast<const float*>(it + (size_t)nd * K::LP);
    static_assert(32 * K::WAVES == (FM >= 48 ? 128 : 256), "receivers per workgroup");
    hipLaunchKernelGGL(knn_donor_mfma_kernel<FM>, dim3(rb, nsp), dim3(64 * K::WAVES), 0, st, (const float*)R,
                       (const unsigned long long*)rmask, nr, rows, (const unsigned long long*)dmask, nd, F, per,
                       (const int*)slot_col, (unsigned long long*)best, (unsigned*)alt, (const int*)cnt, s0, it,
                       (const float*)ny);
  };
  const int FM = knn_mf_fm(F);
  if (FM == 16) go(std::integral_constant<int, 16>{});
  else if (FM == 24) go(std::integral_constant<int, 24>{});
  else if (FM == 32) go(std::integral_constant<int, 32>{});
  else if (FM == 40) go(std::integral_constant<int, 40>{});
  else go(std::integral_constant<int, 48>{});
  launch_check();
}


__device__ __forceinline__ double knn_dist64(const double* __restrict__ x, unsigned long long mr,
                                             const double* __restrict__ y, unsigned long long md, int F);

__global__ __launch_bounds__(256) void knn_ambig_kernel(const unsigned long long* __restrict__ best,
                                                        const unsigned* __restrict__ alt,
                                                        const int* __restrict__ slot_col, int nr, int F,
                                                        const float* __restrict__ Mx, float* __restrict__ thr,
                                                        unsigned long long* __restrict__ dmin,
                                                        int* __restrict__ didx, int* __restrict__ rlist,
                                                        int* __restrict__ counts,
                                                        const double* __restrict__ R64,
                                                        const unsigned long long* __restrict__ rmask,
                                                        const double* __restrict__ D64,
                                                        const unsigned long long* __restrict__ dmask,
                                                        unsigned long long* __restrict__ dwin,
                                                        const int* __restrict__ cnt, int s0) {
  if (cnt != nullptr) {
    if (s0 >= cnt[1]) return;
    nr = cnt[0];
  }
  const int r = blockIdx.x * 256 + threadIdx.x;
  if (r >= nr) return;
  const float mn = Mx[0], Ff = (float)F;
  bool any = false;
#pragma unroll
  for (int k = 0; k < kKnnSlots; ++k) {
    const size_t e = (size_t)r * kKnnSlots + k;
    float t = -1.f;
    const unsigned long long b = best[e];
    if (slot_col[e] >= 0 && b != ~0ull) {
      const float d1 = __uint_as_float((unsigned)(b >> 32));
      const float W = 0x1p-20f * (8.f * mn * sqrtf(Ff * d1) + (Ff + 2.f) * d1) + 0x1p-42f * Ff * Ff * mn * mn;
      const unsigned a = alt[e];
      if (a != 0xFFFFFFFFu && __uint_as_float(a) <= d1 + W) {
        t = d1 + W;
        any = true;
      }
    }
    thr[e] = t;
    unsigned long long w64 = ~0ull;
    int wi = 0x7fffffff;
    if (t >= 0.f) {
      wi = (int)(unsigned)(b & 0xFFFFFFFFull);
      w64 = (unsigned long long)__double_as_longlong(
          knn_dist64(R64 + (size_t)r * F, rmask[r], D64 + (size_t)wi * F, dmask[wi], F));
    }
    dwin[e] = w64;
    dmin[e] = w64;
    didx[e] = wi;
  }
  if (any) rlist[atomicAdd(&counts[0], 1)] = r;
}

#pragma clang fp contract(off)
__device__ __forceinline__ double knn_dist64(const double* __restrict__ x, unsigned long long mr,
                                             const double* __restrict__ y, unsigned long long md, int F) {
  double s = 0.0;
  int present = 0;
  for (int f = 0; f < F; ++f) {
    if (((mr | md) >> f) & 1ull) continue;
    const double t = x[f] - y[f];
    s = s + t * t;
    ++present;
  }
  return present > 0 ? (s * (double)F) / (double)present : INFINITY;
}
#pragma clang fp contract(on)

template <int FMAX, int MODE>
__global__ __launch_bounds__(256) void knn_cand_kernel(
    const float* __restrict__ R, const unsigned long long* __restrict__ rmask, const int* __restrict__ rlist,
    const int* __restrict__ counts, const float* __restrict__ D, const unsigned long long* __restrict__ dmask,
    int nd, int F, int per_split, const int* __restrict__ slot_col, const float* __restrict__ thr,
    const double* __restrict__ R64, const double* __restrict__ D64, unsigned long long* __restrict__ dmin,
    int* __restrict__ didx, const unsigned long long* __restrict__ dwin, int* __restrict__ didx2,
    int* __restrict__ pairs, long long cap, int* __restrict__ pcount) {
  constexpr int LD = (FMAX + 3) / 4 * 4;
  if (MODE != 0 && pcount[1] == 0) return;
  const int nrl = counts[0];
  if ((int)blockIdx.x * 256 >= nrl) return;
  extern __shared__ __attribute__((aligned(16))) float sm[];
  float* ds = sm;
  unsigned long long* dm = (unsigned long long*)(ds + kKnnTile * LD);
  const int li = blockIdx.x * 256 + threadIdx.x;
  const bool active = li < nrl;
  const int r = active ? rlist[li] : 0;
  const int d_begin = blockIdx.y * per_split;
  const int d_end = min(nd, d_begin + per_split);
  float xr[LD];
#pragma unroll
  for (int f = 0; f < LD; ++f) xr[f] = (active && f < F) ? R[(size_t)r * F + f] : 0.f;
  const unsigned long long mr = active ? rmask[r] : 0ull;
  int col[kKnnSlots];
  float th[kKnnSlots];
  unsigned long long need = 0ull;
  float tmax = -1.f;
#pragma unroll
  for (int k = 0; k < kKnnSlots; ++k) {
    const size_t e = (size_t)r * kKnnSlots + k;
    th[k] = active ? thr[e] : -1.f;
    col[k] = (active && th[k] >= 0.f) ? slot_col[e] : -1;
    if (col[k] >= 0) need |= 1ull << col[k];
    tmax = fmaxf(tmax, col[k] >= 0 ? th[k] : -1.f);
  }
  const double* x64 = R64 + (size_t)r * F;
  for (int d0 = d_begin; d0 < d_end; d0 += kKnnTile) {
    __syncthreads();
    const int nt = min(kKnnTile, d_end - d0);
    for (int e = threadIdx.x; e < nt * LD; e += 256) {
      const int rr = e / LD, c = e % LD;
      ds[e] = c < F ? D[(size_t)(d0 + rr) * F + c] : 0.f;
    }
    if (threadIdx.x < nt) dm[threadIdx.x] = dmask[d0 + threadIdx.x];
    __syncthreads();
    if (need == 0ull) continue;
    for (int t = 0; t < nt; ++t) {
      const unsigned long long md = dm[t];
      if ((need & ~md) == 0ull) continue;
      const float4* xd4 = reinterpret_cast<const float4*>(ds + t * LD);
      const unsigned long long both = ~(mr | md);
      const unsigned blo = (unsigned)both, bhi = (unsigned)(both >> 32);
      float s0 = 0.f, s1 = 0.f;
#pragma unroll
      for (int q = 0; q < LD / 4; ++q) {
        if (4 * q < F) {
          const float4 v = xd4[q];
          const unsigned bq = ((4 * q < 32 ? blo >> (4 * q) : bhi >> (4 * q - 32))) & 0xFu;
          const float a = (bq & 1u) ? xr[4 * q] - v.x : 0.f;
          const float b = (bq & 2u) ? xr[4 * q + 1] - v.y : 0.f;
          const float c = (bq & 4u) ? xr[4 * q + 2] - v.z : 0.f;
          const float d = (bq & 8u) ? xr[4 * q + 3] - v.w : 0.f;
          s0 = fmaf(a, a, s0);
          s1 = fmaf(b, b, s1);
          s0 = fmaf(c, c, s0);
          s1 = fmaf(d, d, s1);
        }
      }
      const int present = F - __builtin_popcountll(mr | md);
      if (present <= 0) continue;
      const float dist = fmaxf(s0 + s1, 0.f) * ((float)F / (float)present);
      if (!(dist <= tmax)) continue;
      const int di = d0 + t;
      double d64 = -1.0;
#pragma unroll
      for (int k = 0; k < kKnnSlots; ++k) {
        if (col[k] >= 0 && !((md >> col[k]) & 1ull) && dist <= th[k]) {
          const size_t e = (size_t)r * kKnnSlots + k;
          if constexpr (MODE == 0) {
            const int p = atomicAdd(&pcount[0], 1);
            if (p < cap) {
              pairs[2 * (size_t)p] = (int)e;
              pairs[2 * (size_t)p + 1] = di;
            } else {
              pcount[1] = 1;
            }
          } else {
            if (d64 < 0.0) d64 = knn_dist64(x64, mr, D64 + (size_t)di * F, md, F);
            const unsigned long long key = (unsigned long long)__double_as_longlong(d64);
            if constexpr (MODE == 1) {
              if (key < dwin[e]) atomicMin(&dmin[e], key);
              else if (key == dwin[e]) atomicMin(&didx[e], di);
            } else if (key == dmin[e]) {
              atomicMin(&didx2[e], di);
            }
          }
        }
      }
    }
  }
}

template <int STAGE>
__global__ __launch_bounds__(256) void knn_eval_kernel(const int* __restrict__ pairs, const int* __restrict__ pcount,
                                                       long long cap, const int* __restrict__ slot_col,
                                                       const double* __restrict__ R64,
                                                       const unsigned long long* __restrict__ rmask,
                                                       const double* __restrict__ D64,
                                                       const unsigned long long* __restrict__ dmask, int F,
                                                       unsigned long long* __restrict__ keys,
                                                       unsigned long long* __restrict__ dmin,
                                                       const unsigned long long* __restrict__ dwin,
                                                       int* __restrict__ didx, const float* __restrict__ thr2,
                                                       int* __restrict__ didx2) {
  const long long np = min((long long)pcount[0], cap);
  for (long long p = (long long)blockIdx.x * 256 + threadIdx.x; p < np; p += (long long)gridDim.x * 256) {
    const size_t e = (size_t)pairs[2 * p];
    const int di = pairs[2 * p + 1];
    if constexpr (STAGE == 0) {
      const int r = (int)(e / kKnnSlots);
      const double d64 = knn_dist64(R64 + (size_t)r * F, rmask[r], D64 + (size_t)di * F, dmask[di], F);
      const unsigned long long key = (unsigned long long)__double_as_longlong(d64);
      keys[p] = key;
      if (key < dwin[e]) atomicMin(&dmin[e], key);
      else if (key == dwin[e]) atomicMin(&didx[e], di);
    } else {
      if (thr2[e] >= 0.f && keys[p] == dmin[e]) atomicMin(&didx2[e], di);
    }
  }
}

__global__ __launch_bounds__(256) void knn_pass1_list_kernel(const int* __restrict__ rlist, const int* __restrict__ counts,
                                                             const float* __restrict__ thr,
                                                             const unsigned long long* __restrict__ dmin,
                                                             const unsigned long long* __restrict__ dwin,
                                                             float* __restrict__ thr2, int* __restrict__ didx2,
                                                             int* __restrict__ rlist2, int* __restrict__ counts2) {
  const int nrl = counts[0];
  for (int w = blockIdx.x * 256 + threadIdx.x; w < nrl; w += gridDim.x * 256) {
    const int r = rlist[w];
    bool any = false;
#pragma unroll
    for (int k = 0; k < kKnnSlots; ++k) {
      const size_t e = (size_t)r * kKnnSlots + k;
      const bool need = thr[e] >= 0.f && dmin[e] < dwin[e];
      thr2[e] = need ? thr[e] : -1.f;
      didx2[e] = 0x7fffffff;
      any |= need;
    }
    if (any) rlist2[atomicAdd(&counts2[0], 1)] = r;
  }
}

__global__ __launch_bounds__(256) void knn_commit_kernel(const int* __restrict__ rlist, const int* __restrict__ counts,
                                                         const float* __restrict__ thr, const float* __restrict__ thr2,
                                                         const int* __restrict__ didx, const int* __restrict__ didx2,
                                                         unsigned long long* __restrict__ best) {
  const int nrl = counts[0];
  for (int w = blockIdx.x * 256 + threadIdx.x; w < nrl * kKnnSlots; w += gridDim.x * 256) {
    const size_t e = (size_t)rlist[w / kKnnSlots] * kKnnSlots + w % kKnnSlots;
    if (thr[e] < 0.f) continue;
    const int d = thr2[e] >= 0.f ? didx2[e] : didx[e];
    if (d != 0x7fffffff) best[e] = (best[e] & 0xFFFFFFFF00000000ull) | (unsigned long long)(unsigned)d;
  }
}

static int knn_mf_fm(int F);
template <int FM>
static void knn_cand_mfma(const float* R, const unsigned long long* rmask, int nr, const unsigned long long* dmask,
                          int nd, int F, const int* slot_col, const int* rlist, const int* counts, const float* thr,
                          int* pairs, long long cap, int* pcount, const unsigned short* items, const float* ny,
                          hipStream_t st) {
  using K = KnnMf<FM>;
  const int rpb = 32 * K::WAVES;
  const int rb = (nr + rpb - 1) / rpb;
  int splits = (nd + 16383) / 16384;
  if (splits < 64) splits = 64;
  const int max_splits = (nd + 255) / 256;
  if (splits > max_splits) splits = max_splits;
  if (splits < 1) splits = 1;
  int per = (nd + splits - 1) / splits;
  per = (per + 31) / 32 * 32;
  const int nsp = (nd + per - 1) / per;
  const float* rows = reinterpret_cast<const float*>(items + (size_t)nd * K::LP);
  hipLaunchKernelGGL((knn_donor_mfma_kernel<FM, 1>), dim3(rb, nsp), dim3(64 * K::WAVES), 0, st, R, rmask, nr, rows,
                     dmask, nd, F, per, slot_col, (unsigned long long*)nullptr, (unsigned*)nullptr, counts, 0, items,
                     ny, rlist, thr, pairs, cap, pcount);
}

void knn_refine(uintptr_t R, uintptr_t rmask, int nr, uintptr_t D, uintptr_t dmask, int nd, int F,
                uintptr_t slot_col, uintptr_t best, uintptr_t alt, uintptr_t R64, uintptr_t D64, uintptr_t Mx,
                uintptr_t work, long long cap, uintptr_t cnt, int s0, uintptr_t items, uintptr_t ny,
                uintptr_t stream) {
  HFENS_REQUIRE(F >= 1 && F <= 64, "knn_refine: 1 <= F <= 64");
  HFENS_REQUIRE((work & 7) == 0 && cap >= 1, "knn_refine: work must be 8-byte aligned, cap >= 1");
  if (nr == 0 || nd == 0) return;
  hipStream_t st = as_stream(stream);
  const size_t ns = (size_t)nr * kKnnSlots;
  unsigned long long* keys = (unsigned long long*)work;
  unsigned long long* dmin = keys + cap;
  unsigned long long* dwin = dmin + ns;
  int* didx = (int*)(dwin + ns);
  int* didx2 = didx + ns;
  float* thr = (float*)(didx2 + ns);
  float* thr2 = thr + ns;
  int* pairs = (int*)(thr2 + ns);
  int* rlist = pairs + 2 * cap;
  int* rlist2 = rlist + nr;
  int* counts = rlist2 + nr;
  int* counts2 = counts + 4;
  int* pcount = counts2 + 4;
  HFENS_CHECK(hipMemsetAsync(counts, 0, 12 * sizeof(int), st));
  const int rb = (nr + 255) / 256;
  hipLaunchKernelGGL(knn_ambig_kernel, dim3(rb), dim3(256), 0, st, (const unsigned long long*)best,
                     (const unsigned*)alt, (const int*)slot_col, nr, F, (const float*)Mx, thr, dmin, didx, rlist,
                     counts, (const double*)R64, (const unsigned long long*)rmask, (const double*)D64,
                     (const unsigned long long*)dmask, dwin, (const int*)cnt, s0);
  launch_check();
  int splits = 2048 / rb;
  const int by_range = (nd + 16383) / 16384;
  if (splits < by_range) splits = by_range;
  const int max_splits = (nd + kKnnTile - 1) / kKnnTile;
  if (splits > max_splits) splits = max_splits;
  if (splits < 1) splits = 1;
  int eg = (int)((cap + 255) / 256);
  if (eg > 2048) eg = 2048;
  auto go = [&](auto fm) {
    constexpr int FM = decltype(fm)::value;
    constexpr int LD = (FM + 3) / 4 * 4;
    int per = (nd + splits - 1) / splits;
    per = (per + kKnnTile - 1) / kKnnTile * kKnnTile;
    const int nsp = (nd + per - 1) / per;
    const size_t lds = (size_t)kKnnTile * LD * sizeof(float) + kKnnTile * sizeof(unsigned long long);
    auto cand = [&](auto mode, const int* rl, const int* cn, const float* th) {
      constexpr int MD = decltype(mode)::value;
      hipLaunchKernelGGL((knn_cand_kernel<FM, MD>), dim3(rb, nsp), dim3(256), lds, st, (const float*)R,
                         (const unsigned long long*)rmask, rl, cn, (const float*)D, (const unsigned long long*)dmask,
                         nd, F, per, (const int*)slot_col, th, (const double*)R64, (const double*)D64, dmin, didx,
                         (const unsigned long long*)dwin, didx2, pairs, cap, pcount);
    };
    if (items != 0 && F <= 48) {
      const int fm = knn_mf_fm(F);
      auto mf = [&](auto k) {
        knn_cand_mfma<decltype(k)::value>((const float*)R, (const unsigned long long*)rmask, nr,
                                          (const unsigned long long*)dmask, nd, F, (const int*)slot_col, rlist,
                                          counts, thr, pairs, cap, pcount, (const unsigned short*)items,
                                          (const float*)ny, st);
      };
      if (fm == 16) mf(std::integral_constant<int, 16>{});
      else if (fm == 24) mf(std::integral_constant<int, 24>{});
      else if (fm == 32) mf(std::integral_constant<int, 32>{});
      else if (fm == 40) mf(std::integral_constant<int, 40>{});
      else mf(std::integral_constant<int, 48>{});
      launch_check();
    } else {
      cand(std::integral_constant<int, 0>{}, rlist, counts, thr);
    }
    hipLaunchKernelGGL(knn_eval_kernel<0>, dim3(eg), dim3(256), 0, st, (const int*)pairs, (const int*)pcount, cap,
                       (const int*)slot_col, (const double*)R64, (const unsigned long long*)rmask, (const double*)D64,
                       (const unsigned long long*)dmask, F, keys, dmin, (const unsigned long long*)dwin, didx,
                       (const float*)thr2, didx2);
    cand(std::integral_constant<int, 1>{}, rlist, counts, thr);
    int g1 = rb < 1024 ? rb : 1024;
    hipLaunchKernelGGL(knn_pass1_list_kernel, dim3(g1), dim3(256), 0, st, rlist, counts, thr, dmin,
                       (const unsigned long long*)dwin, thr2, didx2, rlist2, counts2);
    hipLaunchKernelGGL(knn_eval_kernel<1>, dim3(eg), dim3(256), 0, st, (const int*)pairs, (const int*)pcount, cap,
                       (const int*)slot_col, (const double*)R64, (const unsigned long long*)rmask, (const double*)D64,
                       (const unsigned long long*)dmask, F, keys, dmin, (const unsigned long long*)dwin, didx,
                       (const float*)thr2, didx2);
    cand(std::integral_constant<int, 2>{}, rlist2, counts2, thr2);
    launch_check();
  };
  if (F <= 16) go(std::integral_constant<int, 16>{});
  else if (F <= 32) go(std::integral_constant<int, 32>{});
  else if (F <= 40) go(std::integral_constant<int, 40>{});
  else if (F <= 48) go(std::integral_constant<int, 48>{});
  else go(std::integral_constant<int, 64>{});
  int grid = (nr * kKnnSlots + 255) / 256;
  if (grid > 4096) grid = 4096;
  hipLaunchKernelGGL(knn_commit_kernel, dim3(grid), dim3(256), 0, st, rlist, counts, thr, thr2, didx, didx2,
                     (unsigned long long*)best);
  launch_check();
}

__global__ __launch_bounds__(256) void knn_plan_count_kernel(const double* __restrict__ X, long long n, int F,
                                                             int* __restrict__ bcnt, int* __restrict__ cnt) {
  const long long r = (long long)blockIdx.x * 256 + threadIdx.x;
  int m = 0;
  if (r < n)
    for (int f = 0; f < F; ++f) m += isnan(X[r * F + f]) ? 1 : 0;
  const unsigned long long b = __ballot(m > 0);
  int mx = m;
#pragma unroll
  for (int o = 32; o > 0; o >>= 1) mx = max(mx, __shfl_xor(mx, o, kWave));
  __shared__ int wc[4], wm[4], wn[4];
  int nc = m;
#pragma unroll
  for (int o = 32; o > 0; o >>= 1) nc += __shfl_xor(nc, o, kWave);
  const int lane = threadIdx.x & 63, wave = threadIdx.x >> 6;
  if (lane == 0) { wc[wave] = __popcll(b); wm[wave] = mx; wn[wave] = nc; }
  __syncthreads();
  if (threadIdx.x == 0) {
    bcnt[blockIdx.x] = wc[0] + wc[1] + wc[2] + wc[3];
    atomicMax(&cnt[1], max(max(wm[0], wm[1]), max(wm[2], wm[3])));
    atomicAdd(&cnt[2], wn[0] + wn[1] + wn[2] + wn[3]);
  }
}

__global__ __launch_bounds__(1024) void knn_plan_scan_kernel(int* __restrict__ bcnt, int nb, int* __restrict__ cnt) {
  __shared__ int part[1024];
  const int per = (nb + 1023) / 1024;
  const int b0 = threadIdx.x * per;
  int s = 0;
  for (int i = 0; i < per; ++i) s += (b0 + i < nb) ? bcnt[b0 + i] : 0;
  part[threadIdx.x] = s;
  __syncthreads();
  for (int o = 1; o < 1024; o <<= 1) {
    const int v = threadIdx.x >= o ? part[threadIdx.x - o] : 0;
    __syncthreads();
    part[threadIdx.x] += v;
    __syncthreads();
  }
  int run = part[threadIdx.x] - s;
  for (int i = 0; i < per; ++i) {
    if (b0 + i < nb) {
      const int c = bcnt[b0 + i];
      bcnt[b0 + i] = run;
      run += c;
    }
  }
  if (threadIdx.x == 1023) {
    cnt[0] = part[1023];
    cnt[1] = (cnt[1] + kKnnSlots - 1) / kKnnSlots * kKnnSlots;
  }
}

__global__ __launch_bounds__(256) void knn_plan_fill_kernel(const double* __restrict__ X, long long n, int F,
                                                            const double* __restrict__ centre,
                                                            const int* __restrict__ boff, int G,
                                                            long long* __restrict__ rows,
                                                            unsigned long long* __restrict__ rbits,
                                                            int* __restrict__ slot, float* __restrict__ R32,
                                                            double* __restrict__ R64, unsigned* __restrict__ colmax) {
  const long long r = (long long)blockIdx.x * 256 + threadIdx.x;
  unsigned long long bits = 0ull;
  if (r < n)
    for (int f = 0; f < F; ++f) bits |= (isnan(X[r * F + f]) ? 1ull : 0ull) << f;
  const unsigned long long b = __ballot(bits != 0ull);
  const int lane = threadIdx.x & 63, wave = threadIdx.x >> 6;
  __shared__ int wc[4];
  if (lane == 0) wc[wave] = __popcll(b);
  __syncthreads();
  if (bits == 0ull) return;
  int k = boff[blockIdx.x] + __popcll(b & ((1ull << lane) - 1ull));
  for (int w = 0; w < wave; ++w) k += wc[w];
  rows[k] = r;
  rbits[k] = bits;
  int s = 0;
  for (int f = 0; f < F; ++f) {
    const double x = X[r * F + f];
    const bool miss = (bits >> f) & 1ull;
    const float z = miss ? 0.f : (float)(x - centre[f]);
    R32[(size_t)k * F + f] = z;
    R64[(size_t)k * F + f] = miss ? 0.0 : x;
    if (!miss) atomicMax(&colmax[f], __float_as_uint(fabsf(z)));
    if (miss) {
      slot[((size_t)(s / kKnnSlots) * n + k) * kKnnSlots + s % kKnnSlots] = f;
      ++s;
    }
  }
  for (; s < G * kKnnSlots; ++s) slot[((size_t)(s / kKnnSlots) * n + k) * kKnnSlots + s % kKnnSlots] = -1;
}

__global__ void knn_plan_mx_kernel(const float* __restrict__ dmax, const unsigned* __restrict__ colmax, int F,
                                   float* __restrict__ Mx) {
  if (threadIdx.x != 0) return;
  double s = 0.0;
  for (int f = 0; f < F; ++f) {
    const double v = (double)fmaxf(dmax[f], __uint_as_float(colmax[f]));
    s += v * v;
  }
  Mx[0] = (float)sqrt(s);
}

void knn_plan_dev(uintptr_t X, long long n, int F, uintptr_t centre, uintptr_t dmax, uintptr_t rows, uintptr_t rbits,
                  uintptr_t slot, int G, uintptr_t R32, uintptr_t R64, uintptr_t colmax, uintptr_t Mx, uintptr_t cnt,
                  uintptr_t bcnt, uintptr_t stream) {
  HFENS_REQUIRE(F >= 1 && F <= 64 && G * kKnnSlots >= F && n >= 1, "knn_plan_dev: 1 <= F <= 64, G·8 >= F");
  hipStream_t st = as_stream(stream);
  const long long nb = (n + 255) / 256;
  HFENS_REQUIRE(nb <= (1LL << 30), "knn_plan_dev: too many rows");
  HFENS_CHECK(hipMemsetAsync((void*)cnt, 0, 4 * sizeof(int), st));
  HFENS_CHECK(hipMemsetAsync((void*)colmax, 0, (size_t)F * sizeof(unsigned), st));
  hipLaunchKernelGGL(knn_plan_count_kernel, dim3((unsigned)nb), dim3(256), 0, st, (const double*)X, n, F,
                     (int*)bcnt, (int*)cnt);
  hipLaunchKernelGGL(knn_plan_scan_kernel, dim3(1), dim3(1024), 0, st, (int*)bcnt, (int)nb, (int*)cnt);
  hipLaunchKernelGGL(knn_plan_fill_kernel, dim3((unsigned)nb), dim3(256), 0, st, (const double*)X, n, F,
                     (const double*)centre, (const int*)bcnt, G, (long long*)rows, (unsigned long long*)rbits,
                     (int*)slot, (float*)R32, (double*)R64, (unsigned*)colmax);
  hipLaunchKernelGGL(knn_plan_mx_kernel, dim3(1), dim3(64), 0, st, (const float*)dmax, (const unsigned*)colmax, F,
                     (float*)Mx);
  launch_check();
}

__global__ __launch_bounds__(256) void knn_apply_kernel(double* __restrict__ X, long long n, int F,
                                                        const long long* __restrict__ rows,
                                                        const int* __restrict__ slot,
                                                        const unsigned long long* __restrict__ best,
                                                        const double* __restrict__ fitX,
                                                        const double* __restrict__ colmean,
                                                        const int* __restrict__ cnt) {
  const long long k = (long long)blockIdx.x * 256 + threadIdx.x;
  if (k >= cnt[0]) return;
  const long long r = rows[k];
  const int G = cnt[1] / kKnnSlots;
  for (int g = 0; g < G; ++g) {
    for (int j = 0; j < kKnnSlots; ++j) {
      const size_t e = ((size_t)g * n + k) * kKnnSlots + j;
      const int c = slot[e];
      if (c < 0) continue;
      const unsigned long long b = best[e];
      const long long d = b == ~0ull ? -1 : (long long)(b & 0xFFFFFFFFull);
      X[r * F + c] = d >= 0 ? fitX[d * F + c] : colmean[c];
    }
  }
}

void knn_apply(uintptr_t X, long long n, int F, uintptr_t rows, uintptr_t slot, uintptr_t best, uintptr_t fitX,
               uintptr_t colmean, uintptr_t cnt, uintptr_t stream) {
  HFENS_REQUIRE(F >= 1 && F <= 64 && n >= 1, "knn_apply: bad shape");
  hipLaunchKernelGGL(knn_apply_kernel, dim3((unsigned)((n + 255) / 256)), dim3(256), 0, as_stream(stream), (double*)X,
                     n, F, (const long long*)rows, (const int*)slot, (const unsigned long long*)best,
                     (const double*)fitX, (const double*)colmean, (const int*)cnt);
  launch_check();
}

}
```

Before: 606,000.

## Fuse KNN imputation into one batched device call over slot groups

Replaces the per-slot-group Python loop of donor/refine launches with a single host entry that launches each kernel once with the slot groups on blockIdx.z. All scratch buffers now come from one byte allocation with a cached layout, cleared by two memsets, and the MFMA donor item prep is cached per fitted data instead of rebuilt on every transform. This cuts host launch overhead, allocator calls and repeated prep work, at the cost of more complex pointer arithmetic and larger per-group work buffers held at the same time.

```diff
diff --git a/machine-learning-replications_amd/models/imputer.py b/machine-learning-replications_amd/models/imputer.py
--- a/machine-learning-replications_amd/models/imputer.py
+++ b/machine-learning-replications_amd/models/imputer.py
@@ -23,6 +23,35 @@
     LAST_REFINE.append((nr, int(work[o]), int(work[o + 8]), int(work[o + 9]), int(work[o + 4]), float(Mx[0])))
 
 
+_LAYOUT = ("cnt", "colmax", "counts", "zero_end", "Mx", "bcnt", "best", "alt", "ones_end", "rows", "rbits", "slot",
+           "R32", "R64", "work", "wstride", "end")
+_LAYOUTS: dict = {}
+
+
+def planned_layout(n, F, cap):
+    lay = _LAYOUTS.get((n, F, cap))
+    if lay is None:
+        from .. import ops
+        o = np.zeros(len(_LAYOUT), dtype=np.int64)
+        ops.ext().knn_impute_layout(n, F, cap, o.ctypes.data)
+        if len(_LAYOUTS) >= 64:
+            _LAYOUTS.clear()
+        lay = _LAYOUTS[(n, F, cap)] = dict(zip(_LAYOUT, (int(v) for v in o)))
+    return lay
+
+
+def planned_view(buf, lay, name, dtype, shape):
+    nbytes = int(np.prod(shape)) * torch.empty(0, dtype=dtype).element_size()
+    return buf[lay[name]:lay[name] + nbytes].view(dtype).view(*shape)
+
+
+def _planned_debug(buf, lay, n, G):
+    c = planned_view(buf, lay, "counts", torch.int32, (G, 12)).cpu()
+    mx = float(planned_view(buf, lay, "Mx", torch.float32, (1,))[0])
+    for g in range(G):
+        LAST_REFINE.append((n, int(c[g, 0]), int(c[g, 8]), int(c[g, 9]), int(c[g, 4]), mx))
+
+
 def _masks_u64(miss: torch.Tensor) -> torch.Tensor:
     F = miss.shape[1]
     w = (2 ** torch.arange(F, dtype=torch.int64, device=miss.device))
@@ -50,6 +79,7 @@
         cnt = (~self._mask_fit).sum(0).clamp(min=1)
         self._col_mean = fx.sum(0) / cnt
         self._keep_host = None
+        self._mf = None
         return self
 
     def _keep(self):
@@ -95,6 +125,26 @@
         self._fit_prep()
         return self._prep[3], self._prep[4]
 
+    def _fit_mfma_items(self):
+        D32, dm = self._fit_prep()
+        mf = getattr(self, "_mf", None)
+        if mf is None or mf[0] is not self._fit_X:
+            from .. import ops
+            E = ops.ext()
+            nd, F = D32.shape
+            wd = np.zeros(1, dtype=np.int64)
+            E.knn_mfma_item_words(F, wd.ctypes.data)
+            items = torch.empty(nd * int(wd[0]), dtype=torch.int32, device=D32.device)
+            ny = torch.empty(nd, dtype=torch.float32, device=D32.device)
+            E.knn_mfma_prep(D32.data_ptr(), dm.data_ptr(), nd, F, items.data_ptr(), ny.data_ptr(),
+                            ops.stream_ptr(D32.device))
+            mf = self._mf = (self._fit_X, items, ny)
+        return mf[1], mf[2]
+
+    def _use_mfma(self, n):
+        nd, F = self._fit_X.shape
+        return (MFMA_FILTER == "1" or (MFMA_FILTER == "auto" and n * nd >= MFMA_MIN_PAIRS)) and F <= 48 and nd > 0
+
     def _impute_planned_many(self, Xs, streams, defer=False):
         from .smo import _to_dev
         from ..utils.timing import hmark
@@ -104,6 +154,7 @@
         keep = None if keep_h.shape[0] == F else _to_dev(keep_h, dev)
         D32, dm = self._fit_prep()
         D64, dmax = self._fit_prep64()
+        mf = self._fit_mfma_items() if any(X.shape[0] > 0 and self._use_mfma(X.shape[0]) for X in Xs) else None
         main = torch.cuda.current_stream(dev)
         ready = torch.cuda.Event()
         ready.record(main)
@@ -111,16 +162,17 @@
         for i, X in enumerate(Xs):
             st = streams[i] if streams is not None and streams[i] is not None else None
             if st is None:
-                self._impute_planned(X, D32, dm, D64, dmax)
+                self._impute_planned(X, D32, dm, D64, dmax, mf)
                 out.append(X if keep is None else X.index_select(1, keep))
                 hmark("imp_main_enqueued")
             else:
                 def job(i=i, X=X, st=st):
                     st.wait_event(ready)
-                    for t in (X, D32, dm, D64, dmax, self._fit_X, self._col_mean) + ((keep,) if keep is not None else ()):
+                    for t in (X, D32, dm, D64, dmax, self._fit_X, self._col_mean) + (mf or ()) + (
+                            (keep,) if keep is not None else ()):
                         t.record_stream(st)
                     with torch.cuda.device(dev), torch.cuda.stream(st):
-                        self._impute_planned(X, D32, dm, D64, dmax)
+                        self._impute_planned(X, D32, dm, D64, dmax, mf)
                         out[i] = X if keep is None else X.index_select(1, keep)
                 out.append(None)
                 jobs.append(job)
@@ -138,58 +190,29 @@
             return out
         return out, run
 
-    def _impute_planned(self, X, D32, dm, D64, dmax):
+    def _impute_planned(self, X, D32, dm, D64, dmax, mf=None):
         from .. import ops
         E = ops.ext()
         n, F = X.shape
         if n == 0:
-            return
+            return None
         dev = X.device
-        s = ops.stream_ptr(dev)
-        G = -(-F // SLOTS)
         Xc = X if X.is_contiguous() else X.contiguous()
-        i64, i32 = torch.int64, torch.int32
-        rows = torch.empty(n, dtype=i64, device=dev)
-        rbits = torch.empty(n, dtype=i64, device=dev)
-        slot = torch.empty(G, n, SLOTS, dtype=i32, device=dev)
-        R32 = torch.empty(n, F, dtype=torch.float32, device=dev)
-        R64 = torch.empty(n, F, dtype=torch.float64, device=dev)
-        small = torch.empty(F + 1 + 4 + (n + 255) // 256, dtype=i32, device=dev)
-        colmax, Mx, cnt, bcnt = small[:F], small[F:F + 1], small[F + 1:F + 5], small[F + 5:]
-        E.knn_plan_dev(Xc.data_ptr(), n, F, self._col_mean.data_ptr(), dmax.data_ptr(), rows.data_ptr(),
-                       rbits.data_ptr(), slot.data_ptr(), G, R32.data_ptr(), R64.data_ptr(), colmax.data_ptr(),
-                       Mx.data_ptr(), cnt.data_ptr(), bcnt.data_ptr(), s)
-        best = torch.empty(G, n, SLOTS, dtype=i64, device=dev)
-        alt = torch.empty(n, SLOTS, dtype=i32, device=dev)
         cap = max(REFINE_CAP_MIN, REFINE_CAP_PER_ROW * n, 1)
-        work = torch.empty(4 * cap + n * SLOTS * 8 + 2 * n + 12, dtype=i32, device=dev)
-        nd = D32.shape[0]
-        mf = None
-        use_mf = MFMA_FILTER == "1" or (MFMA_FILTER == "auto" and n * nd >= MFMA_MIN_PAIRS)
-        if use_mf and F <= 48 and nd > 0:
-            wd = np.zeros(1, dtype=np.int64)
-            E.knn_mfma_item_words(F, wd.ctypes.data)
-            mf = (torch.empty(nd * int(wd[0]), dtype=torch.int32, device=dev), torch.empty(nd, dtype=torch.float32, device=dev))
-            E.knn_mfma_prep(D32.data_ptr(), dm.data_ptr(), nd, F, mf[0].data_ptr(), mf[1].data_ptr(), s)
-        for g in range(G):
-            if mf is not None:
-                E.knn_donors_mfma(R32.data_ptr(), rbits.data_ptr(), n, D32.data_ptr(), dm.data_ptr(), nd, F,
-                                  slot[g].data_ptr(), best[g].data_ptr(), alt.data_ptr(), cnt.data_ptr(), g * SLOTS,
-                                  mf[0].data_ptr(), mf[1].data_ptr(), s)
-            else:
-                E.knn_donors(R32.data_ptr(), rbits.data_ptr(), n, D32.data_ptr(), dm.data_ptr(), nd, F,
-                             slot[g].data_ptr(), best[g].data_ptr(), alt.data_ptr(), cnt.data_ptr(), g * SLOTS, s)
-            E.knn_refine(R32.data_ptr(), rbits.data_ptr(), n, D32.data_ptr(), dm.data_ptr(), nd, F,
-                         slot[g].data_ptr(), best[g].data_ptr(), alt.data_ptr(), R64.data_ptr(), D64.data_ptr(),
-                         Mx.data_ptr(), work.data_ptr(), cap, cnt.data_ptr(), g * SLOTS,
-                         mf[0].data_ptr() if mf is not None else 0, mf[1].data_ptr() if mf is not None else 0, s)
-            if KNN_DEBUG:
-                _refine_debug(work, cap, n, Mx)
+        lay = planned_layout(n, F, cap)
+        buf = torch.empty(lay["end"], dtype=torch.uint8, device=dev)
+        if mf is None or not self._use_mfma(n):
+            mf = None
         fx = self._fit_X if self._fit_X.is_contiguous() else self._fit_X.contiguous()
-        E.knn_apply(Xc.data_ptr(), n, F, rows.data_ptr(), slot.data_ptr(), best.data_ptr(), fx.data_ptr(),
-                    self._col_mean.data_ptr(), cnt.data_ptr(), s)
+        E.knn_impute_planned(Xc.data_ptr(), n, F, self._col_mean.data_ptr(), dmax.data_ptr(), D32.data_ptr(),
+                             dm.data_ptr(), D64.data_ptr(), D32.shape[0], fx.data_ptr(),
+                             mf[0].data_ptr() if mf is not None else 0, mf[1].data_ptr() if mf is not None else 0,
+                             buf.data_ptr(), buf.numel(), cap, ops.stream_ptr(dev))
+        if KNN_DEBUG:
+            _planned_debug(buf, lay, n, -(-F // SLOTS))
         if Xc is not X:
             X.copy_(Xc)
+        return buf, lay
 
     def _impute_device_many(self, Xs, streams, defer=False):
         F = Xs[0].shape[1]
diff --git a/machine-learning-replications_amd/ops/csrc/decls.inc b/machine-learning-replications_amd/ops/csrc/decls.inc
--- a/machine-learning-replications_amd/ops/csrc/decls.inc
+++ b/machine-learning-replications_amd/ops/csrc/decls.inc
@@ -200,6 +200,10 @@
                         uintptr_t Mx, uintptr_t cnt, uintptr_t bcnt, uintptr_t stream))
 HFENS_OP(knn_apply, (uintptr_t X, long long n, int F, uintptr_t rows, uintptr_t slot, uintptr_t best, uintptr_t fitX,
                      uintptr_t colmean, uintptr_t cnt, uintptr_t stream))
+HFENS_OP(knn_impute_layout, (long long n, int F, long long cap, uintptr_t out))
+HFENS_OP(knn_impute_planned, (uintptr_t X, long long n, int F, uintptr_t centre, uintptr_t dmax, uintptr_t D32,
+                              uintptr_t dmask, uintptr_t D64, int nd, uintptr_t fitX, uintptr_t items, uintptr_t ny,
+                              uintptr_t scratch, long long scratch_bytes, long long cap, uintptr_t stream))
 HFENS_OP(host_store, (uintptr_t src, uintptr_t dst_host, long long n, int elem_bytes, uintptr_t stream))
 HFENS_OP(rbf_f64, (uintptr_t Z, long long l, uintptr_t L, int m, int F, double gamma, uintptr_t out, uintptr_t stream))
 #undef HFENS_OP
diff --git a/machine-learning-replications_amd/ops/csrc/knn.hip b/machine-learning-replications_amd/ops/csrc/knn.hip
--- a/machine-learning-replications_amd/ops/csrc/knn.hip
+++ b/machine-learning-replications_amd/ops/csrc/knn.hip
@@ -1,11 +1,17 @@
 #include "common.h"
 #include <cstdlib>
+#include <cstring>
 #include <type_traits>
 
 namespace hfens {
 
 constexpr int kKnnTile = 256;
 constexpr int kKnnSlots = 8;
+constexpr int kKnnCounts = 12;
+template <class T>
+__device__ __forceinline__ T* knn_grp(T* p, long long bytes) {
+  return reinterpret_cast<T*>(reinterpret_cast<uintptr_t>(p) + bytes);
+}
 
 __device__ __forceinline__ void knn_merge_slots(unsigned long long* best, unsigned* alt, int r,
                                                 const float (&bd)[kKnnSlots], const float (&b2)[kKnnSlots],
@@ -31,6 +37,13 @@
     unsigned long long* __restrict__ best ,
     unsigned* __restrict__ alt ,
     const int* __restrict__ cnt , int s0) {
+  {
+    const size_t go = (size_t)blockIdx.z * nr * kKnnSlots;
+    slot_col += go;
+    best += go;
+    alt += go;
+    s0 += blockIdx.z * kKnnSlots;
+  }
   if (cnt != nullptr) {
     if (s0 >= cnt[1]) return;
     nr = cnt[0];
@@ -142,6 +155,13 @@
     const float* __restrict__ D, const unsigned long long* __restrict__ dmask, int nd, int F,
     int per_split, const int* __restrict__ slot_col, unsigned long long* __restrict__ best,
     unsigned* __restrict__ alt, const int* __restrict__ cnt, int s0) {
+  {
+    const size_t go = (size_t)blockIdx.z * nr * kKnnSlots;
+    slot_col += go;
+    best += go;
+    alt += go;
+    s0 += blockIdx.z * kKnnSlots;
+  }
   if (cnt != nullptr) {
     if (s0 >= cnt[1]) return;
     nr = cnt[0];
@@ -317,13 +337,9 @@
   if (active) knn_merge_slots(best, alt, r, bd, b2, bi);
 }
 
-void knn_donors(uintptr_t R, uintptr_t rmask, int nr, uintptr_t D, uintptr_t dmask, int nd, int F,
-                uintptr_t slot_col, uintptr_t best, uintptr_t alt, uintptr_t cnt, int s0, uintptr_t stream) {
-  HFENS_REQUIRE(F >= 1 && F <= 64, "knn_donors: 1 <= F <= 64 (64-bit missing masks)");
-  if (nr == 0 || nd == 0) return;
-  hipStream_t st = as_stream(stream);
-  HFENS_CHECK(hipMemsetAsync((void*)best, 0xFF, (size_t)nr * kKnnSlots * sizeof(unsigned long long), st));
-  HFENS_CHECK(hipMemsetAsync((void*)alt, 0xFF, (size_t)nr * kKnnSlots * sizeof(unsigned), st));
+static void knn_donors_groups(uintptr_t R, uintptr_t rmask, int nr, uintptr_t D, uintptr_t dmask, int nd, int F,
+                              uintptr_t slot_col, uintptr_t best, uintptr_t alt, uintptr_t cnt, int s0, int G,
+                              hipStream_t st) {
   const int rb = (nr + 255) / 256;
   int splits = 2048 / rb;
   const int by_range = (nd + 16383) / 16384;
@@ -344,17 +360,17 @@
     const size_t lds = direct ? (size_t)kKnnTile * LD * sizeof(float) + kKnnTile * sizeof(unsigned long long)
                               : knn_fast_lds<FM>();
     if (direct)
-      hipLaunchKernelGGL(knn_donor_kernel<FM>, dim3(rb, nsp), dim3(256), lds, st, (const float*)R,
+      hipLaunchKernelGGL(knn_donor_kernel<FM>, dim3(rb, nsp, G), dim3(256), lds, st, (const float*)R,
                          (const unsigned long long*)rmask, nr, (const float*)D,
                          (const unsigned long long*)dmask, nd, F, per, (const int*)slot_col,
                          (unsigned long long*)best, (unsigned*)alt, (const int*)cnt, s0);
     else if (F == LD && !lds_tiles && (D & 15) == 0)
-      hipLaunchKernelGGL((knn_donor_fast_kernel<FM, true>), dim3(rb, nsp), dim3(256), knn_fast_lds_sm<FM>(), st,
+      hipLaunchKernelGGL((knn_donor_fast_kernel<FM, true>), dim3(rb, nsp, G), dim3(256), knn_fast_lds_sm<FM>(), st,
                          (const float*)R, (const unsigned long long*)rmask, nr, (const float*)D,
                          (const unsigned long long*)dmask, nd, F, per, (const int*)slot_col,
                          (unsigned long long*)best, (unsigned*)alt, (const int*)cnt, s0);
     else
-      hipLaunchKernelGGL((knn_donor_fast_kernel<FM, false>), dim3(rb, nsp), dim3(256), lds, st, (const float*)R,
+      hipLaunchKernelGGL((knn_donor_fast_kernel<FM, false>), dim3(rb, nsp, G), dim3(256), lds, st, (const float*)R,
                          (const unsigned long long*)rmask, nr, (const float*)D,
                          (const unsigned long long*)dmask, nd, F, per, (const int*)slot_col,
                          (unsigned long long*)best, (unsigned*)alt, (const int*)cnt, s0);
@@ -365,6 +381,16 @@
   else if (F <= 40) go(std::integral_constant<int, 40>{});
   else if (F <= 48) go(std::integral_constant<int, 48>{});
   else go(std::integral_constant<int, 64>{});
+}
+
+void knn_donors(uintptr_t R, uintptr_t rmask, int nr, uintptr_t D, uintptr_t dmask, int nd, int F,
+                uintptr_t slot_col, uintptr_t best, uintptr_t alt, uintptr_t cnt, int s0, uintptr_t stream) {
+  HFENS_REQUIRE(F >= 1 && F <= 64, "knn_donors: 1 <= F <= 64 (64-bit missing masks)");
+  if (nr == 0 || nd == 0) return;
+  hipStream_t st = as_stream(stream);
+  HFENS_CHECK(hipMemsetAsync((void*)best, 0xFF, (size_t)nr * kKnnSlots * sizeof(unsigned long long), st));
+  HFENS_CHECK(hipMemsetAsync((void*)alt, 0xFF, (size_t)nr * kKnnSlots * sizeof(unsigned), st));
+  knn_donors_groups(R, rmask, nr, D, dmask, nd, F, slot_col, best, alt, cnt, s0, 1, st);
 }
 
 
@@ -426,14 +452,26 @@
     unsigned* __restrict__ alt, const int* __restrict__ cnt, int s0,
     const unsigned short* __restrict__ items, const float* __restrict__ ny_all,
     const int* __restrict__ rlist = nullptr, const float* __restrict__ thr = nullptr,
-    int* __restrict__ pairs = nullptr, long long cap = 0, int* __restrict__ pcount = nullptr) {
+    int* __restrict__ pairs = nullptr, long long cap = 0, int* __restrict__ pcount = nullptr,
+    long long wstride = 0) {
   using K = KnnMf<FM>;
+  slot_col += (size_t)blockIdx.z * nr * kKnnSlots;
   if constexpr (MODE == 1) {
+    cnt += blockIdx.z * kKnnCounts;
+    pcount += blockIdx.z * kKnnCounts;
+    rlist = knn_grp(rlist, blockIdx.z * wstride);
+    thr = knn_grp(thr, blockIdx.z * wstride);
+    pairs = knn_grp(pairs, blockIdx.z * wstride);
     nr = cnt[0];
     if ((int)blockIdx.x * (32 * K::WAVES) >= nr) return;
-  } else if (cnt != nullptr) {
-    if (s0 >= cnt[1]) return;
-    nr = cnt[0];
+  } else {
+    best += (size_t)blockIdx.z * nr * kKnnSlots;
+    alt += (size_t)blockIdx.z * nr * kKnnSlots;
+    s0 += blockIdx.z * kKnnSlots;
+    if (cnt != nullptr) {
+      if (s0 >= cnt[1]) return;
+      nr = cnt[0];
+    }
   }
   constexpr int LD = FM;
   constexpr int NT = 64 * K::WAVES;
@@ -723,15 +761,9 @@
   launch_check();
 }
 
-void knn_donors_mfma(uintptr_t R, uintptr_t rmask, int nr, uintptr_t D, uintptr_t dmask, int nd, int F,
-                     uintptr_t slot_col, uintptr_t best, uintptr_t alt, uintptr_t cnt, int s0, uintptr_t items,
-                     uintptr_t ny, uintptr_t stream) {
-  HFENS_REQUIRE(F >= 1 && F <= 48, "knn_donors_mfma: 1 <= F <= 48");
-  (void)D;
-  if (nr == 0 || nd == 0) return;
-  hipStream_t st = as_stream(stream);
-  HFENS_CHECK(hipMemsetAsync((void*)best, 0xFF, (size_t)nr * kKnnSlots * sizeof(unsigned long long), st));
-  HFENS_CHECK(hipMemsetAsync((void*)alt, 0xFF, (size_t)nr * kKnnSlots * sizeof(unsigned), st));
+static void knn_donors_mfma_groups(uintptr_t R, uintptr_t rmask, int nr, uintptr_t dmask, int nd, int F,
+                                   uintptr_t slot_col, uintptr_t best, uintptr_t alt, uintptr_t cnt, int s0,
+                                   uintptr_t items, uintptr_t ny, int G, hipStream_t st) {
   const int rpb = knn_mf_fm(F) >= 48 ? 128 : 256;
   const int rb = (nr + rpb - 1) / rpb;
   static const int kWgs = getenv("HFENS_KNN_MFMA_WGS") ? atoi(getenv("HFENS_KNN_MFMA_WGS")) : 256;
@@ -752,7 +784,7 @@
     const unsigned short* it = (const unsigned short*)items;
     const float* rows = reinterpret_cast<const float*>(it + (size_t)nd * K::LP);
     static_assert(32 * K::WAVES == (FM >= 48 ? 128 : 256), "receivers per workgroup");
-    hipLaunchKernelGGL(knn_donor_mfma_kernel<FM>, dim3(rb, nsp), dim3(64 * K::WAVES), 0, st, (const float*)R,
+    hipLaunchKernelGGL(knn_donor_mfma_kernel<FM>, dim3(rb, nsp, G), dim3(64 * K::WAVES), 0, st, (const float*)R,
                        (const unsigned long long*)rmask, nr, rows, (const unsigned long long*)dmask, nd, F, per,
                        (const int*)slot_col, (unsigned long long*)best, (unsigned*)alt, (const int*)cnt, s0, it,
                        (const float*)ny);
@@ -764,6 +796,18 @@
   else if (FM == 40) go(std::integral_constant<int, 40>{});
   else go(std::integral_constant<int, 48>{});
   launch_check();
+}
+
+void knn_donors_mfma(uintptr_t R, uintptr_t rmask, int nr, uintptr_t D, uintptr_t dmask, int nd, int F,
+                     uintptr_t slot_col, uintptr_t best, uintptr_t alt, uintptr_t cnt, int s0, uintptr_t items,
+                     uintptr_t ny, uintptr_t stream) {
+  HFENS_REQUIRE(F >= 1 && F <= 48, "knn_donors_mfma: 1 <= F <= 48");
+  (void)D;
+  if (nr == 0 || nd == 0) return;
+  hipStream_t st = as_stream(stream);
+  HFENS_CHECK(hipMemsetAsync((void*)best, 0xFF, (size_t)nr * kKnnSlots * sizeof(unsigned long long), st));
+  HFENS_CHECK(hipMemsetAsync((void*)alt, 0xFF, (size_t)nr * kKnnSlots * sizeof(unsigned), st));
+  knn_donors_mfma_groups(R, rmask, nr, dmask, nd, F, slot_col, best, alt, cnt, s0, items, ny, 1, st);
 }
 
 
@@ -782,7 +826,21 @@
                                                         const double* __restrict__ D64,
                                                         const unsigned long long* __restrict__ dmask,
                                                         unsigned long long* __restrict__ dwin,
-                                                        const int* __restrict__ cnt, int s0) {
+                                                        const int* __restrict__ cnt, int s0, long long wstride) {
+  {
+    const size_t go = (size_t)blockIdx.z * nr * kKnnSlots;
+    const long long wo = blockIdx.z * wstride;
+    best += go;
+    alt += go;
+    slot_col += go;
+    s0 += blockIdx.z * kKnnSlots;
+    thr = knn_grp(thr, wo);
+    dmin = knn_grp(dmin, wo);
+    dwin = knn_grp(dwin, wo);
+    didx = knn_grp(didx, wo);
+    rlist = knn_grp(rlist, wo);
+    counts += blockIdx.z * kKnnCounts;
+  }
   if (cnt != nullptr) {
     if (s0 >= cnt[1]) return;
     nr = cnt[0];
@@ -842,8 +900,22 @@
     int nd, int F, int per_split, const int* __restrict__ slot_col, const float* __restrict__ thr,
     const double* __restrict__ R64, const double* __restrict__ D64, unsigned long long* __restrict__ dmin,
     int* __restrict__ didx, const unsigned long long* __restrict__ dwin, int* __restrict__ didx2,
-    int* __restrict__ pairs, long long cap, int* __restrict__ pcount) {
+    int* __restrict__ pairs, long long cap, int* __restrict__ pcount, int ncap ,
+    long long wstride) {
   constexpr int LD = (FMAX + 3) / 4 * 4;
+  {
+    const long long wo = blockIdx.z * wstride;
+    slot_col += (size_t)blockIdx.z * ncap * kKnnSlots;
+    rlist = knn_grp(rlist, wo);
+    thr = knn_grp(thr, wo);
+    dmin = knn_grp(dmin, wo);
+    didx = knn_grp(didx, wo);
+    dwin = knn_grp(dwin, wo);
+    didx2 = knn_grp(didx2, wo);
+    pairs = knn_grp(pairs, wo);
+    counts += blockIdx.z * kKnnCounts;
+    pcount += blockIdx.z * kKnnCounts;
+  }
   if (MODE != 0 && pcount[1] == 0) return;
   const int nrl = counts[0];
   if ((int)blockIdx.x * 256 >= nrl) return;
@@ -949,7 +1021,18 @@
                                                        unsigned long long* __restrict__ dmin,
                                                        const unsigned long long* __restrict__ dwin,
                                                        int* __restrict__ didx, const float* __restrict__ thr2,
-                                                       int* __restrict__ didx2) {
+                                                       int* __restrict__ didx2, long long wstride) {
+  {
+    const long long wo = blockIdx.z * wstride;
+    pairs = knn_grp(pairs, wo);
+    keys = knn_grp(keys, wo);
+    dmin = knn_grp(dmin, wo);
+    dwin = knn_grp(dwin, wo);
+    didx = knn_grp(didx, wo);
+    thr2 = knn_grp(thr2, wo);
+    didx2 = knn_grp(didx2, wo);
+    pcount += blockIdx.z * kKnnCounts;
+  }
   const long long np = min((long long)pcount[0], cap);
   for (long long p = (long long)blockIdx.x * 256 + threadIdx.x; p < np; p += (long long)gridDim.x * 256) {
     const size_t e = (size_t)pairs[2 * p];
@@ -972,7 +1055,20 @@
                                                              const unsigned long long* __restrict__ dmin,
                                                              const unsigned long long* __restrict__ dwin,
                                                              float* __restrict__ thr2, int* __restrict__ didx2,
-                                                             int* __restrict__ rlist2, int* __restrict__ counts2) {
+                                                             int* __restrict__ rlist2, int* __restrict__ counts2,
+                                                             long long wstride) {
+  {
+    const long long wo = blockIdx.z * wstride;
+    rlist = knn_grp(rlist, wo);
+    thr = knn_grp(thr, wo);
+    dmin = knn_grp(dmin, wo);
+    dwin = knn_grp(dwin, wo);
+    thr2 = knn_grp(thr2, wo);
+    didx2 = knn_grp(didx2, wo);
+    rlist2 = knn_grp(rlist2, wo);
+    counts += blockIdx.z * kKnnCounts;
+    counts2 += blockIdx.z * kKnnCounts;
+  }
   const int nrl = counts[0];
   for (int w = blockIdx.x * 256 + threadIdx.x; w < nrl; w += gridDim.x * 256) {
     const int r = rlist[w];
@@ -992,7 +1088,18 @@
 __global__ __launch_bounds__(256) void knn_commit_kernel(const int* __restrict__ rlist, const int* __restrict__ counts,
                                                          const float* __restrict__ thr, const float* __restrict__ thr2,
                                                          const int* __restrict__ didx, const int* __restrict__ didx2,
-                                                         unsigned long long* __restrict__ best) {
+                                                         unsigned long long* __restrict__ best,
+                                                         int ncap , long long wstride) {
+  {
+    const long long wo = blockIdx.z * wstride;
+    rlist = knn_grp(rlist, wo);
+    thr = knn_grp(thr, wo);
+    thr2 = knn_grp(thr2, wo);
+    didx = knn_grp(didx, wo);
+    didx2 = knn_grp(didx2, wo);
+    counts += blockIdx.z * kKnnCounts;
+    best += (size_t)blockIdx.z * ncap * kKnnSlots;
+  }
   const int nrl = counts[0];
   for (int w = blockIdx.x * 256 + threadIdx.x; w < nrl * kKnnSlots; w += gridDim.x * 256) {
     const size_t e = (size_t)rlist[w / kKnnSlots] * kKnnSlots + w % kKnnSlots;
@@ -1007,7 +1114,7 @@
 static void knn_cand_mfma(const float* R, const unsigned long long* rmask, int nr, const unsigned long long* dmask,
                           int nd, int F, const int* slot_col, const int* rlist, const int* counts, const float* thr,
                           int* pairs, long long cap, int* pcount, const unsigned short* items, const float* ny,
-                          hipStream_t st) {
+                          int G, long long wstride, hipStream_t st) {
   using K = KnnMf<FM>;
   const int rpb = 32 * K::WAVES;
   const int rb = (nr + rpb - 1) / rpb;
@@ -1020,19 +1127,19 @@
   per = (per + 31) / 32 * 32;
   const int nsp = (nd + per - 1) / per;
   const float* rows = reinterpret_cast<const float*>(items + (size_t)nd * K::LP);
-  hipLaunchKernelGGL((knn_donor_mfma_kernel<FM, 1>), dim3(rb, nsp), dim3(64 * K::WAVES), 0, st, R, rmask, nr, rows,
+  hipLaunchKernelGGL((knn_donor_mfma_kernel<FM, 1>), dim3(rb, nsp, G), dim3(64 * K::WAVES), 0, st, R, rmask, nr, rows,
                      dmask, nd, F, per, slot_col, (unsigned long long*)nullptr, (unsigned*)nullptr, counts, 0, items,
-                     ny, rlist, thr, pairs, cap, pcount);
-}
-
-void knn_refine(uintptr_t R, uintptr_t rmask, int nr, uintptr_t D, uintptr_t dmask, int nd, int F,
-                uintptr_t slot_col, uintptr_t best, uintptr_t alt, uintptr_t R64, uintptr_t D64, uintptr_t Mx,
-                uintptr_t work, long long cap, uintptr_t cnt, int s0, uintptr_t items, uintptr_t ny,
-                uintptr_t stream) {
-  HFENS_REQUIRE(F >= 1 && F <= 64, "knn_refine: 1 <= F <= 64");
-  HFENS_REQUIRE((work & 7) == 0 && cap >= 1, "knn_refine: work must be 8-byte aligned, cap >= 1");
-  if (nr == 0 || nd == 0) return;
-  hipStream_t st = as_stream(stream);
+                     ny, rlist, thr, pairs, cap, pcount, wstride);
+}
+
+static long long knn_refine_group_words(long long nr, long long cap) {
+  return 4 * cap + 8 * nr * kKnnSlots + 2 * nr;
+}
+
+static void knn_refine_groups(uintptr_t R, uintptr_t rmask, int nr, uintptr_t D, uintptr_t dmask, int nd, int F,
+                              uintptr_t slot_col, uintptr_t best, uintptr_t alt, uintptr_t R64, uintptr_t D64,
+                              uintptr_t Mx, uintptr_t work, long long cap, int* counts_, long long wstride,
+                              uintptr_t cnt, int s0, uintptr_t items, uintptr_t ny, int G, hipStream_t st) {
   const size_t ns = (size_t)nr * kKnnSlots;
   unsigned long long* keys = (unsigned long long*)work;
   unsigned long long* dmin = keys + cap;
@@ -1044,15 +1151,14 @@
   int* pairs = (int*)(thr2 + ns);
   int* rlist = pairs + 2 * cap;
   int* rlist2 = rlist + nr;
-  int* counts = rlist2 + nr;
+  int* counts = counts_;
   int* counts2 = counts + 4;
   int* pcount = counts2 + 4;
-  HFENS_CHECK(hipMemsetAsync(counts, 0, 12 * sizeof(int), st));
   const int rb = (nr + 255) / 256;
-  hipLaunchKernelGGL(knn_ambig_kernel, dim3(rb), dim3(256), 0, st, (const unsigned long long*)best,
+  hipLaunchKernelGGL(knn_ambig_kernel, dim3(rb, 1, G), dim3(256), 0, st, (const unsigned long long*)best,
                      (const unsigned*)alt, (const int*)slot_col, nr, F, (const float*)Mx, thr, dmin, didx, rlist,
                      counts, (const double*)R64, (const unsigned long long*)rmask, (const double*)D64,
-                     (const unsigned long long*)dmask, dwin, (const int*)cnt, s0);
+                     (const unsigned long long*)dmask, dwin, (const int*)cnt, s0, wstride);
   launch_check();
   int splits = 2048 / rb;
   const int by_range = (nd + 16383) / 16384;
@@ -1071,10 +1177,10 @@
     const size_t lds = (size_t)kKnnTile * LD * sizeof(float) + kKnnTile * sizeof(unsigned long long);
     auto cand = [&](auto mode, const int* rl, const int* cn, const float* th) {
       constexpr int MD = decltype(mode)::value;
-      hipLaunchKernelGGL((knn_cand_kernel<FM, MD>), dim3(rb, nsp), dim3(256), lds, st, (const float*)R,
+      hipLaunchKernelGGL((knn_cand_kernel<FM, MD>), dim3(rb, nsp, G), dim3(256), lds, st, (const float*)R,
                          (const unsigned long long*)rmask, rl, cn, (const float*)D, (const unsigned long long*)dmask,
                          nd, F, per, (const int*)slot_col, th, (const double*)R64, (const double*)D64, dmin, didx,
-                         (const unsigned long long*)dwin, didx2, pairs, cap, pcount);
+                         (const unsigned long long*)dwin, didx2, pairs, cap, pcount, nr, wstride);
     };
     if (items != 0 && F <= 48) {
       const int fm = knn_mf_fm(F);
@@ -1082,7 +1188,7 @@
         knn_cand_mfma<decltype(k)::value>((const float*)R, (const unsigned long long*)rmask, nr,
                                           (const unsigned long long*)dmask, nd, F, (const int*)slot_col, rlist,
                                           counts, thr, pairs, cap, pcount, (const unsigned short*)items,
-                                          (const float*)ny, st);
+                                          (const float*)ny, G, wstride, st);
       };
       if (fm == 16) mf(std::integral_constant<int, 16>{});
       else if (fm == 24) mf(std::integral_constant<int, 24>{});
@@ -1093,18 +1199,18 @@
     } else {
       cand(std::integral_constant<int, 0>{}, rlist, counts, thr);
     }
-    hipLaunchKernelGGL(knn_eval_kernel<0>, dim3(eg), dim3(256), 0, st, (const int*)pairs, (const int*)pcount, cap,
+    hipLaunchKernelGGL(knn_eval_kernel<0>, dim3(eg, 1, G), dim3(256), 0, st, (const int*)pairs, (const int*)pcount, cap,
                        (const int*)slot_col, (const double*)R64, (const unsigned long long*)rmask, (const double*)D64,
                        (const unsigned long long*)dmask, F, keys, dmin, (const unsigned long long*)dwin, didx,
-                       (const float*)thr2, didx2);
+                       (const float*)thr2, didx2, wstride);
     cand(std::integral_constant<int, 1>{}, rlist, counts, thr);
     int g1 = rb < 1024 ? rb : 1024;
-    hipLaunchKernelGGL(knn_pass1_list_kernel, dim3(g1), dim3(256), 0, st, rlist, counts, thr, dmin,
-                       (const unsigned long long*)dwin, thr2, didx2, rlist2, counts2);
-    hipLaunchKernelGGL(knn_eval_kernel<1>, dim3(eg), dim3(256), 0, st, (const int*)pairs, (const int*)pcount, cap,
+    hipLaunchKernelGGL(knn_pass1_list_kernel, dim3(g1, 1, G), dim3(256), 0, st, rlist, counts, thr, dmin,
+                       (const unsigned long long*)dwin, thr2, didx2, rlist2, counts2, wstride);
+    hipLaunchKernelGGL(knn_eval_kernel<1>, dim3(eg, 1, G), dim3(256), 0, st, (const int*)pairs, (const int*)pcount, cap,
                        (const int*)slot_col, (const double*)R64, (const unsigned long long*)rmask, (const double*)D64,
                        (const unsigned long long*)dmask, F, keys, dmin, (const unsigned long long*)dwin, didx,
-                       (const float*)thr2, didx2);
+                       (const float*)thr2, didx2, wstride);
     cand(std::integral_constant<int, 2>{}, rlist2, counts2, thr2);
     launch_check();
   };
@@ -1115,9 +1221,23 @@
   else go(std::integral_constant<int, 64>{});
   int grid = (nr * kKnnSlots + 255) / 256;
   if (grid > 4096) grid = 4096;
-  hipLaunchKernelGGL(knn_commit_kernel, dim3(grid), dim3(256), 0, st, rlist, counts, thr, thr2, didx, didx2,
-                     (unsigned long long*)best);
+  hipLaunchKernelGGL(knn_commit_kernel, dim3(grid, 1, G), dim3(256), 0, st, rlist, counts, thr, thr2, didx, didx2,
+                     (unsigned long long*)best, nr, wstride);
   launch_check();
+}
+
+void knn_refine(uintptr_t R, uintptr_t rmask, int nr, uintptr_t D, uintptr_t dmask, int nd, int F,
+                uintptr_t slot_col, uintptr_t best, uintptr_t alt, uintptr_t R64, uintptr_t D64, uintptr_t Mx,
+                uintptr_t work, long long cap, uintptr_t cnt, int s0, uintptr_t items, uintptr_t ny,
+                uintptr_t stream) {
+  HFENS_REQUIRE(F >= 1 && F <= 64, "knn_refine: 1 <= F <= 64");
+  HFENS_REQUIRE((work & 7) == 0 && cap >= 1, "knn_refine: work must be 8-byte aligned, cap >= 1");
+  if (nr == 0 || nd == 0) return;
+  hipStream_t st = as_stream(stream);
+  int* counts = (int*)work + knn_refine_group_words(nr, cap);
+  HFENS_CHECK(hipMemsetAsync(counts, 0, kKnnCounts * sizeof(int), st));
+  knn_refine_groups(R, rmask, nr, D, dmask, nd, F, slot_col, best, alt, R64, D64, Mx, work, cap, counts, 0, cnt, s0,
+                    items, ny, 1, st);
 }
 
 __global__ __launch_bounds__(256) void knn_plan_count_kernel(const double* __restrict__ X, long long n, int F,
@@ -1220,6 +1340,10 @@
   Mx[0] = (float)sqrt(s);
 }
 
+static void knn_plan_launch(uintptr_t X, long long n, int F, uintptr_t centre, uintptr_t dmax, uintptr_t rows,
+                            uintptr_t rbits, uintptr_t slot, int G, uintptr_t R32, uintptr_t R64, uintptr_t colmax,
+                            uintptr_t Mx, uintptr_t cnt, uintptr_t bcnt, hipStream_t st);
+
 void knn_plan_dev(uintptr_t X, long long n, int F, uintptr_t centre, uintptr_t dmax, uintptr_t rows, uintptr_t rbits,
                   uintptr_t slot, int G, uintptr_t R32, uintptr_t R64, uintptr_t colmax, uintptr_t Mx, uintptr_t cnt,
                   uintptr_t bcnt, uintptr_t stream) {
@@ -1229,6 +1353,13 @@
   HFENS_REQUIRE(nb <= (1LL << 30), "knn_plan_dev: too many rows");
   HFENS_CHECK(hipMemsetAsync((void*)cnt, 0, 4 * sizeof(int), st));
   HFENS_CHECK(hipMemsetAsync((void*)colmax, 0, (size_t)F * sizeof(unsigned), st));
+  knn_plan_launch(X, n, F, centre, dmax, rows, rbits, slot, G, R32, R64, colmax, Mx, cnt, bcnt, st);
+}
+
+static void knn_plan_launch(uintptr_t X, long long n, int F, uintptr_t centre, uintptr_t dmax, uintptr_t rows,
+                            uintptr_t rbits, uintptr_t slot, int G, uintptr_t R32, uintptr_t R64, uintptr_t colmax,
+                            uintptr_t Mx, uintptr_t cnt, uintptr_t bcnt, hipStream_t st) {
+  const long long nb = (n + 255) / 256;
   hipLaunchKernelGGL(knn_plan_count_kernel, dim3((unsigned)nb), dim3(256), 0, st, (const double*)X, n, F,
                      (int*)bcnt, (int*)cnt);
   hipLaunchKernelGGL(knn_plan_scan_kernel, dim3(1), dim3(1024), 0, st, (int*)bcnt, (int)nb, (int*)cnt);
@@ -1272,4 +1403,69 @@
   launch_check();
 }
 
-}
+struct KnnImputeLayout {
+  long long cnt, colmax, counts, zero_end, Mx, bcnt, best, alt, ones_end, rows, rbits, slot, R32, R64, work, wstride,
+      end;
+};
+constexpr int kKnnLayoutWords = sizeof(KnnImputeLayout) / sizeof(long long);
+
+static KnnImputeLayout knn_impute_layout_of(long long n, int F, long long cap) {
+  const long long G = (F + kKnnSlots - 1) / kKnnSlots, ns = n * kKnnSlots;
+  auto up = [](long long v) { return (v + 15) & ~15LL; };
+  KnnImputeLayout L;
+  long long o = 0;
+  L.cnt = o, o += 4 * 4;
+  L.colmax = o, o += 4LL * F;
+  L.counts = o, o += 4LL * kKnnCounts * G;
+  L.zero_end = o, o = up(o);
+  L.Mx = o, o += 4;
+  L.bcnt = o, o = up(o + 4 * ((n + 255) / 256));
+  L.best = o, o += 8 * G * ns;
+  L.alt = o, o += 4 * G * ns;
+  L.ones_end = o, o = up(o);
+  L.rows = o, o = up(o + 8 * n);
+  L.rbits = o, o = up(o + 8 * n);
+  L.slot = o, o = up(o + 4 * G * ns);
+  L.R32 = o, o = up(o + 4 * n * F);
+  L.R64 = o, o = up(o + 8 * n * F);
+  L.work = o;
+  L.wstride = 4 * knn_refine_group_words(n, cap);
+  L.end = up(o + G * L.wstride);
+  return L;
+}
+
+void knn_impute_layout(long long n, int F, long long cap, uintptr_t out) {
+  HFENS_REQUIRE(F >= 1 && F <= 64 && n >= 1 && cap >= 1, "knn_impute_layout: bad shape");
+  const KnnImputeLayout L = knn_impute_layout_of(n, F, cap);
+  static_assert(kKnnLayoutWords == 17, "KnnImputeLayout");
+  std::memcpy(reinterpret_cast<void*>(out), &L, sizeof(L));
+}
+
+void knn_impute_planned(uintptr_t X, long long n, int F, uintptr_t centre, uintptr_t dmax, uintptr_t D32,
+                        uintptr_t dmask, uintptr_t D64, int nd, uintptr_t fitX, uintptr_t items, uintptr_t ny,
+                        uintptr_t scratch, long long scratch_bytes, long long cap, uintptr_t stream) {
+  HFENS_REQUIRE(F >= 1 && F <= 64 && n >= 1 && n < (1LL << 28) && nd >= 0 && cap >= 1,
+                "knn_impute_planned: 1 <= F <= 64, 1 <= n < 2^28, cap >= 1");
+  HFENS_REQUIRE(items == 0 || F <= 48, "knn_impute_planned: the matrix-core filter takes F <= 48");
+  const KnnImputeLayout L = knn_impute_layout_of(n, F, cap);
+  HFENS_REQUIRE((scratch & 15) == 0 && scratch_bytes >= L.end, "knn_impute_planned: scratch too small or misaligned");
+  hipStream_t st = as_stream(stream);
+  const int G = (F + kKnnSlots - 1) / kKnnSlots, nr = (int)n;
+  HFENS_CHECK(hipMemsetAsync((void*)(scratch + L.cnt), 0, (size_t)(L.zero_end - L.cnt), st));
+  HFENS_CHECK(hipMemsetAsync((void*)(scratch + L.best), 0xFF, (size_t)(L.ones_end - L.best), st));
+  const uintptr_t cnt = scratch + L.cnt, slot = scratch + L.slot, best = scratch + L.best, alt = scratch + L.alt;
+  const uintptr_t rbits = scratch + L.rbits, R32 = scratch + L.R32, R64 = scratch + L.R64, Mx = scratch + L.Mx;
+  knn_plan_launch(X, n, F, centre, dmax, scratch + L.rows, rbits, slot, G, R32, R64, scratch + L.colmax, Mx, cnt,
+                  scratch + L.bcnt, st);
+  if (nd > 0) {
+    if (items != 0)
+      knn_donors_mfma_groups(R32, rbits, nr, dmask, nd, F, slot, best, alt, cnt, 0, items, ny, G, st);
+    else
+      knn_donors_groups(R32, rbits, nr, D32, dmask, nd, F, slot, best, alt, cnt, 0, G, st);
+    knn_refine_groups(R32, rbits, nr, D32, dmask, nd, F, slot, best, alt, R64, D64, Mx, scratch + L.work, cap,
+                      (int*)(scratch + L.counts), L.wstride, cnt, 0, items, ny, G, st);
+  }
+  knn_apply(X, n, F, scratch + L.rows, slot, best, fitX, centre, cnt, stream);
+}
+
+}
```

After: 615,700 (median of 4 runs). Within noise of the previous version (+1.6%).
